# wtomin/MIMAMO-Net

Measured on AMD Instinct MI355X. Metric: face-frames/sec end-to-end (phase-diff + ResNet50 + 2-stream GRU), 64-frame clips, higher is better.
Workload: dtype f32

## Files before the change

### mimamo-net_amd/__init__.py

```python
__version__ = "0.1.0"

_LAZY = {
    "Phase_Difference_Extractor": ".phase_difference_extractor",
    "SCFpyr_PyTorch": ".scfpyr",
    "Steerable_Pyramid_Phase": ".phase_difference_extractor",
    "Resnet50_Extractor": ".resnet50_extractor",
    "Two_Stream_RNN": ".mimamo_net",
    "Tester": ".tester",
    "Snippet_Sampler": ".sampler",
    "Image_Sampler": ".sampler",
}


def __getattr__(name):
    if name in _LAZY:
        import importlib
        mod = importlib.import_module(_LAZY[name], __name__)
        return getattr(mod, name)
    raise AttributeError(name)
```

### mimamo-net_amd/csrc/conv.h

```cpp
#pragma once
#include "mm_common.h"

namespace mm {

struct ConvParams {
    const float* in;
    const float* w;
    const float* bias;
    const float* res;
    const float* post_scale;
    const float* post_shift;
    float* out;
    int B, H, W, Cin, in_cstride, in_coff;
    int Ho, Wo, Cout, out_cstride, out_coff;
    int res_cstride, res_coff;
    int res_rs, RH, RW;
    int kh, kw, stride, pad;
    int K, Kpad;
    int korder;
    int relu;
    int force_tile;
    int ablate;
    int Cin_real;
    int batch;
    int64_t in_bstride, w_bstride, out_bstride;
    int M, tiles_m, tiles_n;
    int m_end;
    int m_off;
    const float* in2;
    int H2, W2, C2, in2_cstride, in2_coff, stride2;
    int sched1x1;
    int no_sched;
    int use_panel;
    int x3;
    const unsigned short* w3;
    int64_t w3_plane;
    unsigned div_hw_mul, div_hw_sh, div_wo_mul, div_wo_sh;
    int hpool;
};

int conv_forward(const ConvParams& p, hipStream_t stream);
int bf16x3_split_weights(const float* w, unsigned short* out, int64_t n, hipStream_t stream);
bool conv_panel_supported(const ConvParams& p);
int conv_panel_forward(const ConvParams& p, hipStream_t stream);
int conv_panel_rows(const ConvParams& p);
int conv_panel_per_cu(const ConvParams& p);

int nchw_to_nhwc(const float* in, float* out, int64_t N, int C, int HW, int cstride, int coff, int cpad, hipStream_t s);
int nchw3_to_bordered_nhwc3(const float* in, float* out, int64_t N, int S, int pad, hipStream_t s);
int maxpool3x3s2(const float* in, float* out, int64_t N, int H, int W, int C, int Ho, int Wo, hipStream_t s);
int maxpool_reduce64(const float* in, const float* w, const float* bias, float* x_out, float* y_out, int64_t N, int H, int W, int Ho, int Wo,
                     int relu, hipStream_t s, int hp = 0);
int avgpool_hw(const float* in, float* out, int64_t N, int HW, int C, int out_cstride, int out_coff, int relu, hipStream_t s);
int wino_input_transform(const float* x, float* V, int B, int H, int W, int C, int m, hipStream_t s, int x_channels = 0);
int wino_output_transform(const float* M, const float* bias, float* y, int B, int H, int W, int Cout, int relu, int m, hipStream_t s);

int wino_gemm_output_fused(const float* V, const float* U, const float* bias, float* y, int B, int H, int W, int Cin, int Cout,
                           int relu, int shape, hipStream_t s, int generic_loop = 0);
int wino_gemm_output_fused_inc(const float* V, const float* U, const float* bias, const float* W2, const float* bias2, const float* res,
                               float* out, int B, int H, int W, int Cin, int Cout, int C2, int relu, hipStream_t s, int generic_loop = 0,
                               const float* next_w = nullptr, const float* next_bias = nullptr, float* next_out = nullptr, int shape = 0);
bool wino_fused_inc_supported(int64_t ntile, int Cin, int Cout, int C2);
int wino_gemm_output_fused_incproj(const float* V, const float* U, const float* bias, const float* W2, const float* bias2, const float* x,
                                   float* out, int B, int H, int W, int Cin, int Cout, int C2, int relu, hipStream_t s, int generic_loop = 0);
bool wino_fused_supported(int64_t ntile, int Cin, int Cout);

int gru_gates(const float* gi, int gi_stride, int gi_off, const float* gh, const float* bhh, const float* h_prev,
              int hp_stride, int hp_off, float* h_out, int out_stride, int out_off, int64_t Bt, int H, hipStream_t s);

}
```

### mimamo-net_amd/csrc/nets.hip

```cpp
#include <cmath>
#include <cstdlib>
#include <cstring>
#include <new>
#include "conv.h"

namespace mm {

struct Layer {
    float *w = nullptr, *bias = nullptr, *ps = nullptr, *pt = nullptr;
    float* wino_u = nullptr;
    float* wino_u4 = nullptr;
    int cin = 0, cin_p = 0, cout = 0, k = 1, stride = 1, pad = 0, K = 0, Kpad = 0, relu = 0, korder = 0;
    int wino_cin = 0;
    int tile = 0;
    unsigned short *w3 = nullptr, *wino_u4_3 = nullptr;
};

struct DeviceArena {
    std::vector<void*> ptrs;
    int upload(const std::vector<float>& h, float** out) {
        *out = nullptr;
        if (h.empty()) return MM_OK;
        void* d = nullptr;
        MM_HIP(hipMalloc(&d, h.size() * sizeof(float)));
        ptrs.push_back(d);
        MM_HIP(hipMemcpy(d, h.data(), h.size() * sizeof(float), hipMemcpyHostToDevice));
        *out = (float*)d;
        return MM_OK;
    }
    void release() {
        for (void* p : ptrs) (void)hipFree(p);
        ptrs.clear();
    }
};

struct BN {
    const float *gamma, *beta, *mean, *var;
};

static int make_layer(DeviceArena& A, Layer& L, const float* w, const float* bias, int cout, int cin, int k, int stride,
                      int pad, int relu, const BN* fold, const BN* post, float eps, bool wino = false, bool packed3 = false,
                      int wino_pad = 0) {
    if (packed3) {
        if (cin != 3) return MM_ERR_INVALID_ARG;
        const int RG = (k * 3 + 3) / 4 * 4;
        L.cin = 3; L.cin_p = 3; L.cout = cout; L.k = k; L.stride = stride; L.pad = 0; L.relu = relu;
        L.K = k * RG; L.Kpad = (L.K + 15) / 16 * 16; L.korder = 2;
        std::vector<float> hw((size_t)cout * L.Kpad, 0.f), hb(cout, 0.f);
        for (int o = 0; o < cout; ++o) {
            double sc = 1.0, sh = 0.0;
            if (fold) {
                sc = (double)fold->gamma[o] / std::sqrt((double)fold->var[o] + (double)eps);
                sh = (double)fold->beta[o] - (double)fold->mean[o] * sc;
            }
            for (int c = 0; c < 3; ++c)
                for (int r = 0; r < k; ++r)
                    for (int q = 0; q < k; ++q)
                        hw[(size_t)o * L.Kpad + r * RG + q * 3 + c] = (float)((double)w[(((size_t)o * 3 + c) * k + r) * k + q] * sc);
            hb[o] = (float)((bias ? (double)bias[o] : 0.0) * sc + sh);
        }
        int rc = A.upload(hw, &L.w);
        if (rc == MM_OK) rc = A.upload(hb, &L.bias);
        return rc;
    }
    L.cin = cin;
    L.cin_p = (cin + 3) / 4 * 4;
    L.cout = cout;
    L.k = k;
    L.stride = stride;
    L.pad = pad;
    L.relu = relu;
    L.K = k * k * L.cin_p;
    L.Kpad = (L.K + 15) / 16 * 16;
    L.korder = (k > 1 && L.cin_p % 16 == 0) ? 1 : 0;
    std::vector<float> hw((size_t)cout * L.Kpad, 0.f), hb(cout, 0.f);
    for (int o = 0; o < cout; ++o) {
        double sc = 1.0, sh = 0.0;
        if (fold) {
            sc = (double)fold->gamma[o] / std::sqrt((double)fold->var[o] + (double)eps);
            sh = (double)fold->beta[o] - (double)fold->mean[o] * sc;
        }
        for (int c = 0; c < cin; ++c)
            for (int r = 0; r < k; ++r)
                for (int s = 0; s < k; ++s)
                {
                    const size_t kidx = L.korder == 0 ? (size_t)(r * k + s) * L.cin_p + c
                                                      : ((size_t)((c / 16) * k + r) * k + s) * 16 + c % 16;
                    hw[(size_t)o * L.Kpad + kidx] = (float)((double)w[(((size_t)o * cin + c) * k + r) * k + s] * sc);
                }
        hb[o] = (float)((bias ? (double)bias[o] : 0.0) * sc + sh);
    }
    int rc = A.upload(hw, &L.w);
    if (rc == MM_OK) rc = A.upload(hb, &L.bias);
    const int wcin = wino_pad > 0 ? (cin + wino_pad - 1) / wino_pad * wino_pad : cin;
    if (rc == MM_OK && wino && k == 3 && stride == 1 && pad == 1 && wcin % 16 == 0 && cin >= 64 && cin % 4 == 0 && cout % 4 == 0) {
        L.wino_cin = wcin;
        static const double G[4][3] = {{1, 0, 0}, {0.5, 0.5, 0.5}, {0.5, -0.5, 0.5}, {0, 0, 1}};
        std::vector<float> hu((size_t)16 * cout * wcin, 0.f);
        for (int o = 0; o < cout; ++o) {
            const double sc = fold ? (double)fold->gamma[o] / std::sqrt((double)fold->var[o] + (double)eps) : 1.0;
            for (int c = 0; c < cin; ++c) {
                double g[3][3], t[4][3];
                for (int r = 0; r < 3; ++r)
                    for (int q = 0; q < 3; ++q) g[r][q] = (double)w[(((size_t)o * cin + c) * 3 + r) * 3 + q] * sc;
                for (int i = 0; i < 4; ++i)
                    for (int q = 0; q < 3; ++q) t[i][q] = G[i][0] * g[0][q] + G[i][1] * g[1][q] + G[i][2] * g[2][q];
                for (int i = 0; i < 4; ++i)
                    for (int j = 0; j < 4; ++j)
                        hu[((size_t)(i * 4 + j) * cout + o) * wcin + c] = (float)(t[i][0] * G[j][0] + t[i][1] * G[j][1] + t[i][2] * G[j][2]);
            }
        }
        rc = A.upload(hu, &L.wino_u);
        static const double G4[6][3] = {{0.25, 0, 0}, {-1.0 / 6, -1.0 / 6, -1.0 / 6}, {-1.0 / 6, 1.0 / 6, -1.0 / 6},
                                        {1.0 / 24, 1.0 / 12, 1.0 / 6}, {1.0 / 24, -1.0 / 12, 1.0 / 6}, {0, 0, 1}};
        std::vector<float> hu4((size_t)36 * cout * wcin, 0.f);
        for (int o = 0; o < cout && rc == MM_OK; ++o) {
            const double sc = fold ? (double)fold->gamma[o] / std::sqrt((double)fold->var[o] + (double)eps) : 1.0;
            for (int c = 0; c < cin; ++c) {
                double g[3][3], t[6][3];
                for (int r = 0; r < 3; ++r)
                    for (int q = 0; q < 3; ++q) g[r][q] = (double)w[(((size_t)o * cin + c) * 3 + r) * 3 + q] * sc;
                for (int i = 0; i < 6; ++i)
                    for (int q = 0; q < 3; ++q) t[i][q] = G4[i][0] * g[0][q] + G4[i][1] * g[1][q] + G4[i][2] * g[2][q];
                for (int i = 0; i < 6; ++i)
                    for (int j = 0; j < 6; ++j)
                        hu4[((size_t)(i * 6 + j) * cout + o) * wcin + c] = (float)(t[i][0] * G4[j][0] + t[i][1] * G4[j][1] + t[i][2] * G4[j][2]);
            }
        }
        if (rc == MM_OK) rc = A.upload(hu4, &L.wino_u4);
    }
    if (rc == MM_OK && post) {
        std::vector<float> ps(cout), pt(cout);
        for (int o = 0; o < cout; ++o) {
            const double sc = (double)post->gamma[o] / std::sqrt((double)post->var[o] + (double)eps);
            ps[o] = (float)sc;
            pt[o] = (float)((double)post->beta[o] - (double)post->mean[o] * sc);
        }
        rc = A.upload(ps, &L.ps);
        if (rc == MM_OK) rc = A.upload(pt, &L.pt);
    }
    return rc;
}

static int make_layer_dual(DeviceArena& A, Layer& L, const float* w1, const BN& bn1, int c1, const float* w2, const BN& bn2, int c2,
                           int cout, float eps) {
    if (c1 % 16 || c2 % 16) return MM_ERR_UNSUPPORTED;
    L.cin = c1; L.cin_p = c1; L.cout = cout; L.k = 1; L.stride = 1; L.pad = 0; L.relu = 1; L.korder = 0;
    L.K = L.Kpad = c1 + c2;
    std::vector<float> hw((size_t)cout * L.K), hb(cout);
    for (int o = 0; o < cout; ++o) {
        const double s1 = (double)bn1.gamma[o] / std::sqrt((double)bn1.var[o] + (double)eps);
        const double s2 = (double)bn2.gamma[o] / std::sqrt((double)bn2.var[o] + (double)eps);
        for (int c = 0; c < c1; ++c) hw[(size_t)o * L.K + c] = (float)((double)w1[(size_t)o * c1 + c] * s1);
        for (int c = 0; c < c2; ++c) hw[(size_t)o * L.K + c1 + c] = (float)((double)w2[(size_t)o * c2 + c] * s2);
        hb[o] = (float)(((double)bn1.beta[o] - (double)bn1.mean[o] * s1) + ((double)bn2.beta[o] - (double)bn2.mean[o] * s2));
    }
    int rc = A.upload(hw, &L.w);
    if (rc == MM_OK) rc = A.upload(hb, &L.bias);
    return rc;
}

constexpr int kX3MinK = 512;

static int run_layer(const Layer& L, const float* in, int B, int H, int W, int in_cstride, int in_coff, float* out,
                     int out_cstride, int out_coff, const float* res, int res_cstride, hipStream_t s, int* Ho_ = nullptr,
                     int* Wo_ = nullptr, int x3 = 0, int no_sched = 0, int hpool = 0, int use_panel = 0, int stride_ov = 0, int res_rs = 0,
                     int RH = 0, int RW = 0) {
    const int stride = stride_ov > 0 && L.k == 1 ? stride_ov : L.stride;
    ConvParams p;
    std::memset(&p, 0, sizeof(p));
    p.in = in; p.w = L.w; p.bias = L.bias; p.res = res; p.post_scale = L.ps; p.post_shift = L.pt; p.out = out;
    p.B = B; p.H = H; p.W = W; p.Cin = L.cin_p; p.in_cstride = in_cstride; p.in_coff = in_coff;
    p.Ho = (H + 2 * L.pad - L.k) / stride + 1;
    p.Wo = (W + 2 * L.pad - L.k) / stride + 1;
    p.Cout = L.cout; p.out_cstride = out_cstride; p.out_coff = out_coff;
    p.res_cstride = res_cstride; p.res_coff = 0;
    p.res_rs = res_rs; p.RH = RH; p.RW = RW;
    p.kh = L.k; p.kw = L.k; p.stride = stride; p.pad = L.pad;
    p.K = L.K; p.Kpad = L.Kpad; p.relu = L.relu; p.Cin_real = L.cin; p.korder = L.korder; p.force_tile = L.tile;
    p.x3 = x3 && L.k == 1 && L.Kpad >= kX3MinK;
    p.w3 = p.x3 ? L.w3 : nullptr; p.w3_plane = (int64_t)L.cout * L.Kpad;
    p.no_sched = no_sched;
    p.hpool = hpool;
    p.use_panel = use_panel;
    if (Ho_) *Ho_ = p.Ho;
    if (Wo_) *Wo_ = p.Wo;
    return conv_forward(p, s);
}

static int run_layer_dual(const Layer& L, const float* in, int B, int H, int W, const float* in2, int H2, int W2, int C2, int stride2,
                          float* out, hipStream_t s, int x3 = 0, int no_sched = 0) {
    ConvParams p;
    std::memset(&p, 0, sizeof(p));
    p.in = in; p.w = L.w; p.bias = L.bias; p.out = out;
    p.B = B; p.H = H; p.W = W; p.Cin = L.cin; p.in_cstride = L.cin; p.Ho = H; p.Wo = W;
    p.Cout = L.cout; p.out_cstride = L.cout; p.kh = 1; p.kw = 1; p.stride = 1;
    p.K = L.K; p.Kpad = L.Kpad; p.relu = 1; p.Cin_real = L.K;
    p.in2 = in2; p.H2 = H2; p.W2 = W2; p.C2 = C2; p.in2_cstride = C2; p.stride2 = stride2;
    p.x3 = x3 && L.Kpad >= kX3MinK;
    p.w3 = p.x3 ? L.w3 : nullptr; p.w3_plane = (int64_t)L.cout * L.Kpad;
    p.no_sched = no_sched;
    return conv_forward(p, s);
}

static int g_wino_fused_max_cin = 256;
static int g_wino_fused_shape = 0;

static int run_layer_wino(const Layer& L, const float* in, int B, int H, int W, float* out, float* V, float* M, int m, hipStream_t s,
                          const Layer* inc = nullptr, const float* inc_res = nullptr, float* inc_out = nullptr, bool inc_two_src = false,
                          int x3 = 0, int generic_loop = 0, int no_sched = 0, const Layer* next = nullptr, float* next_out = nullptr,
                          int inc_shape = 0) {
    const int mt = m == 5 ? 4 : m;
    const int TH = (H + mt - 1) / mt, TW = (W + mt - 1) / mt, npos = (mt + 2) * (mt + 2);
    const int64_t ntile = (int64_t)B * TH * TW;
    if (ntile > 0x7fffffff) return MM_ERR_INVALID_ARG;
    const bool fused = m == 5;
    if (fused) m = 4;
    const int wc = L.wino_cin;
    if (wc != L.cin_p && m != 4) return MM_ERR_UNSUPPORTED;
    if (!M && !(fused && wino_fused_supported(ntile, wc, L.cout))) return MM_ERR_UNSUPPORTED;
    if (inc && !(fused && inc->k == 1 && inc->stride == 1 && inc->Kpad == (inc_two_src ? 2 : 1) * L.cout && inc->korder == 0 && inc->relu &&
                 !inc->ps && (!inc_two_src || L.cout == 64) && wino_fused_inc_supported(ntile, wc, L.cout, inc->cout)))
        return MM_ERR_UNSUPPORTED;
    if (next && !(inc && !inc_two_src && L.cout == 64 && inc->cout == 256 && next_out && next->k == 1 && next->stride == 1 && next->pad == 0 &&
                  next->cin_p == 256 && next->Kpad == 256 && next->cout == 64 && next->korder == 0 && next->relu && !next->ps && next->bias))
        return MM_ERR_UNSUPPORTED;
    int rc = wino_input_transform(in, V, B, H, W, wc, m, s, L.cin_p);
    if (rc != MM_OK) return rc;
    if (inc && inc_two_src)
        return wino_gemm_output_fused_incproj(V, L.wino_u4, L.bias, inc->w, inc->bias, inc_res, inc_out, B, H, W, wc, L.cout, inc->cout,
                                              L.relu, s, generic_loop);
    if (inc)
        return wino_gemm_output_fused_inc(V, L.wino_u4, L.bias, inc->w, inc->bias, inc_res, inc_out, B, H, W, wc, L.cout, inc->cout,
                                          L.relu, s, generic_loop, next ? next->w : nullptr, next ? next->bias : nullptr, next_out, inc_shape);
    if (fused) {
        rc = wino_gemm_output_fused(V, L.wino_u4, L.bias, out, B, H, W, wc, L.cout, L.relu, g_wino_fused_shape, s, generic_loop);
        if (rc != MM_ERR_UNSUPPORTED) return rc;
    }
    if (!M) return MM_ERR_UNSUPPORTED;
    ConvParams p;
    std::memset(&p, 0, sizeof(p));
    p.in = V; p.w = m == 4 ? L.wino_u4 : L.wino_u; p.out = M;
    p.B = (int)ntile; p.H = 1; p.W = 1; p.Cin = wc; p.in_cstride = wc; p.Ho = 1; p.Wo = 1;
    p.Cout = L.cout; p.out_cstride = L.cout; p.kh = 1; p.kw = 1; p.stride = 1; p.K = wc; p.Kpad = wc; p.Cin_real = wc;
    p.batch = npos; p.in_bstride = ntile * wc; p.w_bstride = (int64_t)L.cout * wc; p.out_bstride = ntile * L.cout;
    p.x3 = x3 && wc >= kX3MinK;
    p.w3 = (p.x3 && m == 4) ? L.wino_u4_3 : nullptr; p.w3_plane = (int64_t)npos * L.cout * wc;
    p.no_sched = no_sched;
    rc = conv_forward(p, s);
    if (rc != MM_OK) return rc;
    return wino_output_transform(M, L.bias, out, B, H, W, L.cout, L.relu, m, s);
}

struct Bump {
    char* base;
    int64_t off = 0, cap;
    Bump(void* b, int64_t c) : base((char*)b), cap(c) {}
    float* take(int64_t floats) {
        const int64_t bytes = (floats * 4 + 255) / 256 * 256;
        float* p = (float*)(base + off);
        off += bytes;
        return p;
    }
    static int64_t size_of(int64_t floats) { return (floats * 4 + 255) / 256 * 256; }
};

static const int kStages[4][4] = {{3, 64, 256, 1}, {4, 128, 512, 2}, {6, 256, 1024, 2}, {3, 512, 2048, 2}};

struct Bottleneck {
    Layer proj, reduce, conv3, increase;
    Layer inc_proj;
    int proj_stride;
    bool has_proj;
};

}

struct mm_resnet50 {
    mm::DeviceArena arena;
    mm::Layer stem;
    mm::Layer stem3;
    std::vector<mm::Bottleneck> blocks;
    int ceil_mode;
    int winograd;
    int fuse_proj;
    int fuse_pool;
    int no_sched;
    int use_panel;
    int wf_generic;
    int precision;
    int fuse_next;
    int inc_shape;
    int fuse_inc;
    int stage_tail;
    int tail_fused;
    int device;
};

struct mm_head {
    mm::DeviceArena arena;
    std::vector<mm::Layer> mlp;
    int feat_dim, mlp_max;
    mm::Layer conv[6], fc1, fc2, transform, gru_ih[2], gru_hh[2][2], classifier;
    float* bhh[2][2];
    int winograd;
    int no_sched;
    int pc;
    int pcp;
    int device;
};

namespace mm {

static int64_t resnet_blob_floats() {
    int64_t n = 64 * 3 * 49 + 4 * 64;
    int cin = 64;
    for (auto& st : kStages)
        for (int b = 0; b < st[0]; ++b) {
            const int mid = st[1], cout = st[2];
            if (b == 0) n += (int64_t)cout * cin + 4 * cout;
            n += (int64_t)mid * cin + 4 * mid;
            n += (int64_t)mid * mid * 9 + 4 * mid;
            n += (int64_t)cout * mid + 4 * cout;
            cin = cout;
        }
    return n;
}

static const int64_t kRsIn4 = 224 * 224 * 4, kRsBig = 112 * 112 * 64, kRsMid = 56 * 56 * 128;
static const int64_t kRsWino = 36 * 14 * 14 * 64;

static const int kMlpPublished[3] = {2048, 256, 256};

static bool mlp_units_ok(int n_units, const int* units) {
    if (n_units < 2 || n_units > 16 || !units || units[n_units - 1] != 256) return false;
    for (int i = 0; i < n_units; ++i)
        if (units[i] <= 0 || units[i] % 4 || units[i] > 65536) return false;
    return true;
}

static bool phase_channels_ok(int pc) { return pc >= 2 && pc <= 256 && pc % 2 == 0; }
static int pad4(int c) { return (c + 3) / 4 * 4; }

static int64_t head_blob_floats(int n_units, const int* units, int pc = 24) {
    int64_t n = 0;
    auto lin = [&](int o, int i) { n += (int64_t)o * i + o; };
    auto bn = [&](int c) { n += 4 * c; };
    for (int i = 1; i < n_units; ++i) { lin(units[i], units[i - 1]); bn(units[i]); }
    const int ch[3][2] = {{pc, 64}, {64 + pc, 128}, {128, 256}};
    for (auto& c : ch) { n += (int64_t)c[1] * c[0] * 9 + c[1]; bn(c[1]); n += (int64_t)c[1] * c[1] * 9 + c[1]; bn(c[1]); }
    lin(256, 256); bn(256); lin(256, 256); bn(256); lin(1, 256); bn(1);
    lin(256, 512); bn(256);
    n += 4 * (384 * 256 + 384 * 128 + 384 + 384);
    lin(2, 256); bn(2);
    return n;
}

}

extern "C" {

int mm_conv2d_nhwc(const float* in, const float* w, const float* bias, const float* residual, const float* post_scale,
                   const float* post_shift, float* out, int B, int H, int W, int Cin, int in_cstride, int in_coff,
                   int Cout, int out_cstride, int out_coff, int res_cstride, int kh, int kw, int stride, int pad,
                   int relu, int tile, int korder, void* stream) {
    using namespace mm;
    if (!in || !w || !out || B < 0 || H <= 0 || W <= 0 || Cin <= 0 || Cout <= 0 || kh <= 0 || kw <= 0 || stride <= 0 ||
        pad < 0 || tile < 0)
        return MM_ERR_INVALID_ARG;
#ifdef MM_MEASURE
    if (tile > 2047) return MM_ERR_INVALID_ARG;
#else
    if (tile > 5) return MM_ERR_INVALID_ARG;
#endif
    if ((post_scale == nullptr) != (post_shift == nullptr)) return MM_ERR_INVALID_ARG;
    ConvParams p;
    std::memset(&p, 0, sizeof(p));
    p.in = in; p.w = w; p.bias = bias; p.res = residual; p.post_scale = post_scale; p.post_shift = post_shift; p.out = out;
    p.B = B; p.H = H; p.W = W; p.Cin = Cin; p.in_cstride = in_cstride; p.in_coff = in_coff;
    p.Ho = (H + 2 * pad - kh) / stride + 1;
    p.Wo = (W + 2 * pad - kw) / stride + 1;
    if (p.Ho <= 0 || p.Wo <= 0 || (int64_t)B * p.Ho * p.Wo > 0x7fffffff) return MM_ERR_INVALID_ARG;
    p.Cout = Cout; p.out_cstride = out_cstride; p.out_coff = out_coff; p.res_cstride = res_cstride;
    p.kh = kh; p.kw = kw; p.stride = stride; p.pad = pad;
    p.K = kh * kw * Cin; p.Kpad = (p.K + 15) / 16 * 16; p.relu = relu; p.force_tile = tile; p.korder = korder;
    {
        const char* cp = getenv("MM_CONV_PANEL");
        p.use_panel = cp ? (atoi(cp) == 1 ? 1 : atoi(cp) == 2 ? 2 : 0) : 0;
    }
    return conv_forward(p, (hipStream_t)stream);
}

int64_t mm_resnet50_blob_floats(void) { return mm::resnet_blob_floats(); }

int mm_resnet50_create(mm_resnet50_t** out, const float* blob, int64_t n_floats, int stride_on_first_1x1,
                       int maxpool_ceil_mode, float bn_eps) {
    using namespace mm;
    if (!out) return MM_ERR_INVALID_ARG;
    *out = nullptr;
    if (!blob || n_floats != resnet_blob_floats()) return MM_ERR_INVALID_ARG;
    int ndev = 0;
    if (hipGetDeviceCount(&ndev) != hipSuccess || ndev == 0) return MM_ERR_NO_DEVICE;
    mm_resnet50* h = new (std::nothrow) mm_resnet50();
    if (!h) return MM_ERR_INVALID_ARG;
    h->ceil_mode = maxpool_ceil_mode;
    h->device = current_device_or(0);
    const float* p = blob;
    int rc = MM_OK;
    h->winograd = 1;
    h->precision = 0;
    {
        const char* wk = getenv("MM_WF_KSL");
        h->wf_generic = wk ? atoi(wk) == 0 : 0;
        const char* cs = getenv("MM_CONV_SCHED");
        h->no_sched = cs ? atoi(cs) == 0 : 0;
        const char* cp = getenv("MM_CONV_PANEL");
        h->use_panel = cp ? (atoi(cp) == 1 ? 1 : atoi(cp) == 2 ? 2 : 0) : 0;
        const char* fp = getenv("MM_FUSE_PROJ");
        h->fuse_proj = fp ? atoi(fp) : 1;
        const char* fpl = getenv("MM_FUSE_POOL");
        h->fuse_pool = fpl ? atoi(fpl) : 2;
        const char* fi = getenv("MM_FUSE_INC");
        h->fuse_inc = fi ? atoi(fi) : 3;
        const char* fn = getenv("MM_FUSE_NEXT");
        h->fuse_next = fn ? atoi(fn) : 0;
        const char* is = getenv("MM_INC1_SHAPE");
        h->inc_shape = is ? atoi(is) : 0;
        const char* tl = getenv("MM_STAGE_TAIL");
        h->stage_tail = tl ? atoi(tl) != 0 : 1;
        const char* tf = getenv("MM_STAGE_TAIL_FUSED");
        h->tail_fused = tf ? atoi(tf) & 3 : 3;
    }
    auto conv_bn = [&](Layer& L, int cout, int cin, int k, int stride, int pad, int relu) {
        const float* w = p;
        p += (int64_t)cout * cin * k * k;
        BN bn{p, p + cout, p + 2 * cout, p + 3 * cout};
        p += 4 * cout;
        if (rc == MM_OK) rc = make_layer(h->arena, L, w, nullptr, cout, cin, k, stride, pad, relu, &bn, nullptr, bn_eps, true);
    };
    {
        const float* w = p;
        BN bn{p + 64 * 3 * 49, p + 64 * 3 * 49 + 64, p + 64 * 3 * 49 + 128, p + 64 * 3 * 49 + 192};
        rc = make_layer(h->arena, h->stem3, w, nullptr, 64, 3, 7, 2, 0, 1, &bn, nullptr, bn_eps, false, true);
    }
    conv_bn(h->stem, 64, 3, 7, 2, 3, 1);
#ifdef MM_MEASURE
    if (const char* st = getenv("MM_STEM_TILE")) {
        const int t = atoi(st);
        if (t >= 0 && t <= 4) h->stem.tile = h->stem3.tile = t;
    }
#endif
    int cin = 64;
    for (auto& st : kStages)
        for (int b = 0; b < st[0]; ++b) {
            const int mid = st[1], cout = st[2], s = b == 0 ? st[3] : 1;
            const int s1 = stride_on_first_1x1 ? s : 1, s3 = stride_on_first_1x1 ? 1 : s;
            h->blocks.emplace_back();
            Bottleneck& B = h->blocks.back();
            B.has_proj = b == 0;
            B.proj_stride = s;
            const float* w_proj = p;
            if (b == 0) conv_bn(B.proj, cout, cin, 1, s, 0, 0);
            conv_bn(B.reduce, mid, cin, 1, s1, 0, 1);
            conv_bn(B.conv3, mid, mid, 3, s3, 1, 1);
            const float* w_inc = p;
            conv_bn(B.increase, cout, mid, 1, 1, 0, 1);
            if (b == 0 && rc == MM_OK) {
                const float* q1 = w_inc + (int64_t)cout * mid;
                const float* q2 = w_proj + (int64_t)cout * cin;
                const BN bn1{q1, q1 + cout, q1 + 2 * cout, q1 + 3 * cout}, bn2{q2, q2 + cout, q2 + 2 * cout, q2 + 3 * cout};
                const int rd = make_layer_dual(h->arena, B.inc_proj, w_inc, bn1, mid, w_proj, bn2, cin, cout, bn_eps);
                if (rd != MM_OK && rd != MM_ERR_UNSUPPORTED) rc = rd;
            }
            cin = cout;
        }
    if (rc != MM_OK) {
        h->arena.release();
        delete h;
        return rc;
    }
    *out = h;
    return MM_OK;
}

int mm_resnet50_destroy(mm_resnet50_t* h) {
    if (!h) return MM_OK;
    h->arena.release();
    delete h;
    return MM_OK;
}

int64_t mm_resnet50_workspace_bytes(mm_resnet50_t* h, int64_t batch) {
    using namespace mm;
    if (!h || batch < 0) return MM_ERR_INVALID_ARG;
    return Bump::size_of(batch * kRsIn4) + 3 * Bump::size_of(batch * kRsBig) + 2 * Bump::size_of(batch * kRsMid) +
           2 * Bump::size_of(batch * kRsWino);
}

int mm_resnet50_set_winograd(mm_resnet50_t* h, int enable) {
    if (!h) return MM_ERR_INVALID_ARG;
    if (enable != 0 && enable != 1 && enable != 2 && enable != 4 && enable != 5) return MM_ERR_INVALID_ARG;
    h->winograd = enable;
#ifdef MM_MEASURE
    const char* mc = getenv("MM_WF_MAX_CIN");
    if (mc) mm::g_wino_fused_max_cin = atoi(mc);
    const char* sh = getenv("MM_WINO_FUSED_SHAPE");
    mm::g_wino_fused_shape = sh ? atoi(sh) : 0;
#endif
    return MM_OK;
}

static int ensure_x3_weights(mm_resnet50_t* h) {
    using namespace mm;
    const char* e = getenv("MM_X3_PRESPLIT");
    if (!e || atoi(e) != 1) return MM_OK;
    auto split = [&](const float* w, int64_t n, unsigned short** out) -> int {
        if (*out || !w || n <= 0 || n % 16) return MM_OK;
        void* d = nullptr;
        MM_HIP(hipMalloc(&d, (size_t)n * 3 * sizeof(unsigned short)));
        h->arena.ptrs.push_back(d);
        const int rc = bf16x3_split_weights(w, (unsigned short*)d, n, nullptr);
        if (rc != MM_OK) return rc;
        *out = (unsigned short*)d;
        return MM_OK;
    };
    for (auto& Bk : h->blocks) {
        for (Layer* L : {&Bk.proj, &Bk.reduce, &Bk.increase, &Bk.inc_proj})
            if (L->w && L->k == 1 && L->Kpad >= kX3MinK && L->cout % 256 == 0) {
                const int rc = split(L->w, (int64_t)L->cout * L->Kpad, &L->w3);
                if (rc != MM_OK) return rc;
            }
        Layer& C = Bk.conv3;
        if (C.wino_u4 && C.wino_cin >= kX3MinK && C.cout % 256 == 0) {
            const int rc = split(C.wino_u4, (int64_t)36 * C.cout * C.wino_cin, &C.wino_u4_3);
            if (rc != MM_OK) return rc;
        }
    }
    MM_HIP(hipDeviceSynchronize());
    return MM_OK;
}

int mm_resnet50_set_precision(mm_resnet50_t* h, int mode) {
    if (!h || (mode != 0 && mode != 1)) return MM_ERR_INVALID_ARG;
    if (mode == 1) {
        MM_CHECK_DEVICE(h);
        const int rc = ensure_x3_weights(h);
        if (rc != MM_OK) return rc;
    }
    h->precision = mode;
    return MM_OK;
}

int mm_resnet50_forward(mm_resnet50_t* h, const float* images, int nchw, int64_t batch, float* out, void* workspace,
                        int64_t workspace_bytes, void* stream_) {
    using namespace mm;
    if (!h || batch < 0 || (batch > 0 && (!images || !out || !workspace))) return MM_ERR_INVALID_ARG;
    if (batch == 0) return MM_OK;
    if (batch > 40000) return MM_ERR_INVALID_ARG;
    MM_CHECK_DEVICE(h);
    if (workspace_bytes < mm_resnet50_workspace_bytes(h, batch)) return MM_ERR_WORKSPACE;
    hipStream_t s = (hipStream_t)stream_;
    const int B = (int)batch;
    Bump ws(workspace, workspace_bytes);
    float* in4 = ws.take(batch * kRsIn4);
    float* big[3] = {ws.take(batch * kRsBig), ws.take(batch * kRsBig), ws.take(batch * kRsBig)};
    float* y1 = ws.take(batch * kRsMid);
    float* y2 = ws.take(batch * kRsMid);
    float* wv = ws.take(batch * kRsWino);
    float* wm = ws.take(batch * kRsWino);
    int rc;
    const float* x0 = images;
    int H = 224, W = 224, Ho, Wo;
    const mm::Layer& R0 = h->blocks.front().reduce;
    const bool pooled_reduce = h->fuse_pool && R0.k == 1 && R0.stride == 1 && R0.pad == 0 && R0.cin_p == 64 && R0.cout == 64 && R0.Kpad == 64 &&
                               R0.korder == 0 && !R0.ps;
    const bool hpool = pooled_reduce && h->fuse_pool >= 2 && nchw;
    if (nchw) {
        if (nchw == 1) {
            rc = nchw3_to_bordered_nhwc3(images, in4, batch, 224, 3, s);
            if (rc != MM_OK) return rc;
            x0 = in4;
        }
        rc = run_layer(h->stem3, x0, B, 230, 230, 3, 0, big[0], 64, 0, nullptr, 0, s, &Ho, &Wo, 0, h->no_sched, hpool);
    } else {
        rc = run_layer(h->stem, x0, B, H, W, 4, 0, big[0], 64, 0, nullptr, 0, s, &Ho, &Wo, 0, h->no_sched);
    }
    if (rc != MM_OK) return rc;
    if (Ho != 112 || Wo != 112) return MM_ERR_UNSUPPORTED;
    H = Ho; W = Wo;
    if (h->ceil_mode) {
        Ho = (H - 3 + 1) / 2 + 1; Wo = (W - 3 + 1) / 2 + 1;
        if ((Ho - 1) * 2 >= H) --Ho;
        if ((Wo - 1) * 2 >= W) --Wo;
    } else {
        Ho = (H - 3) / 2 + 1; Wo = (W - 3) / 2 + 1;
    }
    if (pooled_reduce)
        rc = maxpool_reduce64(big[0], R0.w, R0.bias, big[1], y1, batch, H, W, Ho, Wo, R0.relu, s, hpool);
    else
        rc = maxpool3x3s2(big[0], big[1], batch, H, W, 64, Ho, Wo, s);
    if (rc != MM_OK) return rc;
    H = Ho; W = Wo;
    int xi = 1;
    int C = 64;
    const int x3 = h->precision == 1, ns = h->no_sched;
    bool reduce_done = false;
    bool xc = false;
    for (size_t bi = 0; bi < h->blocks.size(); ++bi) {
        const Bottleneck& Bk = h->blocks[bi];
        const Bottleneck* Nx = bi + 1 < h->blocks.size() ? &h->blocks[bi + 1] : nullptr;
        float* x = big[xi];
        float* sc = big[(xi + 1) % 3];
        float* o = big[(xi + 2) % 3];
        int H1, W1, H2, W2, H3, W3;
        const float* resid = x;
        const bool dual = Bk.has_proj && h->fuse_proj && Bk.inc_proj.w;
        const bool tail_blk = !Bk.has_proj && Nx && Nx->has_proj && Nx->proj_stride == 2 && Nx->reduce.k == 1 && Nx->reduce.stride == 2 &&
                              Nx->reduce.pad == 0 && Nx->proj.k == 1 && Nx->proj.pad == 0 && Bk.increase.k == 1 && Bk.increase.stride == 1 &&
                              Bk.increase.pad == 0;
        bool tail = tail_blk && h->stage_tail && !h->use_panel;
        const bool tail_unfuse = tail_blk && !(h->tail_fused & (Bk.conv3.cout == 64 ? 1 : 2));
        const int sov = xc ? 1 : 0;
        if (Bk.has_proj && !dual) {
            rc = run_layer(Bk.proj, x, B, H, W, C, 0, sc, Bk.proj.cout, 0, nullptr, 0, s, nullptr, nullptr, x3, ns, 0, 0, sov);
            if (rc != MM_OK) return rc;
            resid = sc;
        }
        if ((pooled_reduce && bi == 0) || reduce_done) {
            H1 = H; W1 = W;
            reduce_done = false;
        } else {
            rc = run_layer(Bk.reduce, x, B, H, W, C, 0, y1, Bk.reduce.cout, 0, nullptr, 0, s, &H1, &W1, x3, ns, 0, 0, sov);
            if (rc != MM_OK) return rc;
        }
        const int wm_ = h->winograd == 1 ? (Bk.conv3.cin <= g_wino_fused_max_cin ? 5 : 4) : h->winograd;
        const int wt_ = wm_ == 5 ? 4 : wm_;
        bool inc_done = false;
        if (wm_ && Bk.conv3.wino_u &&
            (int64_t)(wt_ + 2) * (wt_ + 2) * ((H1 + wt_ - 1) / wt_) * ((W1 + wt_ - 1) / wt_) * Bk.conv3.cin <= kRsWino) {
            rc = MM_ERR_UNSUPPORTED;
            if (wm_ == 5 && h->fuse_inc && !Bk.has_proj && !tail_unfuse && (Bk.conv3.cout == 64 || h->fuse_inc >= 3)) {
                const bool nx = h->fuse_next && Bk.conv3.cout == 64 && Nx && !Nx->has_proj && Nx->reduce.stride == 1;
                if (nx) {
                    rc = run_layer_wino(Bk.conv3, y1, B, H1, W1, nullptr, wv, nullptr, 5, s, &Bk.increase, x, o, false, 0, h->wf_generic, 0, &Nx->reduce, y1,
                                        h->inc_shape);
                    reduce_done = rc == MM_OK;
                }
                if (!nx || rc == MM_ERR_UNSUPPORTED)
                    rc = run_layer_wino(Bk.conv3, y1, B, H1, W1, nullptr, wv, nullptr, 5, s, &Bk.increase, x, o, false, 0, h->wf_generic, 0, nullptr, nullptr,
                                        h->inc_shape);
                inc_done = rc == MM_OK;
            } else if (wm_ == 5 && h->fuse_inc >= 2 && dual && Bk.proj_stride == 1 && C == Bk.conv3.cout && H1 == H && W1 == W) {
                rc = run_layer_wino(Bk.conv3, y1, B, H1, W1, nullptr, wv, nullptr, 5, s, &Bk.inc_proj, x, o, true, 0, h->wf_generic);
                inc_done = rc == MM_OK;
            }
            if (rc == MM_ERR_UNSUPPORTED) rc = run_layer_wino(Bk.conv3, y1, B, H1, W1, y2, wv, wm, wm_, s, nullptr, nullptr, nullptr, false, x3, h->wf_generic, ns);
            H2 = H1; W2 = W1;
        } else {
            rc = run_layer(Bk.conv3, y1, B, H1, W1, Bk.reduce.cout, 0, y2, Bk.conv3.cout, 0, nullptr, 0, s, &H2, &W2, 0, ns);
        }
        if (rc != MM_OK) return rc;
        if (inc_done) {
            H3 = H2; W3 = W2;
            tail = false;
        } else if (dual) {
            rc = run_layer_dual(Bk.inc_proj, y2, B, H2, W2, x, H, W, C, xc ? 1 : Bk.proj_stride, o, s, x3, ns);
            H3 = H2; W3 = W2;
        } else if (tail) {
            rc = run_layer(Bk.increase, y2, B, H2, W2, Bk.conv3.cout, 0, o, Bk.increase.cout, 0, resid, Bk.increase.cout, s, &H3, &W3, x3, ns, 0,
                           h->use_panel, 2, 2, H2, W2);
        } else {
            rc = run_layer(Bk.increase, y2, B, H2, W2, Bk.conv3.cout, 0, o, Bk.increase.cout, 0, resid, Bk.increase.cout, s, &H3, &W3, x3, ns, 0, h->use_panel);
        }
        if (rc != MM_OK) return rc;
        H = H3; W = W3; C = Bk.increase.cout;
        xc = tail;
        xi = (xi + 2) % 3;
    }
    if (H != 7 || W != 7) return MM_ERR_UNSUPPORTED;
    return avgpool_hw(big[xi], out, batch, H * W, C, C, 0, 1, s);
}

int64_t mm_head_blob_floats(void) { return mm::head_blob_floats(3, mm::kMlpPublished); }

int64_t mm_head_blob_floats_mlp(int n_units, const int* units) {
    return mm::mlp_units_ok(n_units, units) ? mm::head_blob_floats(n_units, units) : (int64_t)MM_ERR_INVALID_ARG;
}

int mm_head_create(mm_head_t** out, const float* blob, int64_t n_floats) {
    return mm_head_create_mlp(out, blob, n_floats, 3, mm::kMlpPublished);
}

int mm_head_create_mlp(mm_head_t** out, const float* blob, int64_t n_floats, int n_units, const int* units) {
    return mm_head_create_cfg(out, blob, n_floats, n_units, units, 12);
}

int64_t mm_head_blob_floats_cfg(int n_units, const int* units, int num_phase) {
    if (!mm::mlp_units_ok(n_units, units) || num_phase < 1) return (int64_t)MM_ERR_INVALID_ARG;
    if (!mm::phase_channels_ok(2 * num_phase)) return (int64_t)MM_ERR_UNSUPPORTED;
    return mm::head_blob_floats(n_units, units, 2 * num_phase);
}

int mm_head_create_cfg(mm_head_t** out, const float* blob, int64_t n_floats, int n_units, const int* units, int num_phase) {
    using namespace mm;
    if (!out) return MM_ERR_INVALID_ARG;
    *out = nullptr;
    const int pc = 2 * num_phase;
    if (!mlp_units_ok(n_units, units)) return MM_ERR_INVALID_ARG;
    if (num_phase < 1) return MM_ERR_INVALID_ARG;
    if (!phase_channels_ok(pc)) return MM_ERR_UNSUPPORTED;
    if (!blob || n_floats != head_blob_floats(n_units, units, pc)) return MM_ERR_INVALID_ARG;
    int ndev = 0;
    if (hipGetDeviceCount(&ndev) != hipSuccess || ndev == 0) return MM_ERR_NO_DEVICE;
    mm_head* h = new (std::nothrow) mm_head();
    if (!h) return MM_ERR_INVALID_ARG;
    h->device = current_device_or(0);
    h->pc = pc;
    h->pcp = pad4(pc);
    const float eps = 1e-5f;
    const float* p = blob;
    int rc = MM_OK;
    auto take = [&](int64_t n) { const float* q = p; p += n; return q; };
    auto take_bn = [&](int c) { BN b{p, p + c, p + 2 * c, p + 3 * c}; p += 4 * c; return b; };
    auto lin_bn_relu = [&](Layer& L, int o, int i) {
        const float* w = take((int64_t)o * i); const float* b = take(o); BN bn = take_bn(o);
        if (rc == MM_OK) rc = make_layer(h->arena, L, w, b, o, i, 1, 1, 0, 1, &bn, nullptr, eps);
    };
    auto conv_bn_relu = [&](Layer& L, int o, int i, int stride, bool wino) {
        const float* w = take((int64_t)o * i * 9); const float* b = take(o); BN bn = take_bn(o);
        if (rc == MM_OK) rc = make_layer(h->arena, L, w, b, o, i, 3, stride, 1, 1, &bn, nullptr, eps, wino && i <= 128, false, 64);
    };
    auto lin_relu_bn = [&](Layer& L, int o, int i) {
        const float* w = take((int64_t)o * i); const float* b = take(o); BN bn = take_bn(o);
        if (rc == MM_OK) rc = make_layer(h->arena, L, w, b, o, i, 1, 1, 0, 1, nullptr, &bn, eps);
    };
    {
        const char* e = getenv("MM_HEAD_WINOGRAD");
        h->winograd = e ? atoi(e) : 1;
        const char* cs = getenv("MM_CONV_SCHED");
        h->no_sched = cs ? atoi(cs) == 0 : 0;
    }
    h->feat_dim = units[0];
    h->mlp_max = 256;
    h->mlp.resize(n_units - 1);
    for (int i = 1; i < n_units; ++i) {
        lin_bn_relu(h->mlp[i - 1], units[i], units[i - 1]);
        if (units[i] > h->mlp_max) h->mlp_max = units[i];
    }
    const int ch[3][2] = {{pc, 64}, {64 + pc, 128}, {128, 256}};
    for (int i = 0; i < 3; ++i) {
        conv_bn_relu(h->conv[2 * i], ch[i][1], ch[i][0], 1, i >= 1);
        conv_bn_relu(h->conv[2 * i + 1], ch[i][1], ch[i][1], 2, false);
    }
    lin_relu_bn(h->fc1, 256, 256);
    lin_relu_bn(h->fc2, 256, 256);
    take(256 + 1); take_bn(1);
    lin_relu_bn(h->transform, 256, 512);
    for (int l = 0; l < 2 && rc == MM_OK; ++l) {
        std::vector<float> wih(768 * 256), bih(768);
        for (int d = 0; d < 2; ++d) {
            const float* w_ih = take(384 * 256); const float* w_hh = take(384 * 128);
            const float* b_ih = take(384); const float* b_hh = take(384);
            std::memcpy(wih.data() + (size_t)d * 384 * 256, w_ih, sizeof(float) * 384 * 256);
            std::memcpy(bih.data() + (size_t)d * 384, b_ih, sizeof(float) * 384);
            if (rc == MM_OK) rc = make_layer(h->arena, h->gru_hh[l][d], w_hh, b_hh, 384, 128, 1, 1, 0, 0, nullptr, nullptr, eps);
            std::vector<float> bh(b_hh, b_hh + 384);
            if (rc == MM_OK) rc = h->arena.upload(bh, &h->bhh[l][d]);
        }
        if (rc == MM_OK) rc = make_layer(h->arena, h->gru_ih[l], wih.data(), bih.data(), 768, 256, 1, 1, 0, 0, nullptr, nullptr, eps);
    }
    {
        const float* w = take(2 * 256); const float* b = take(2); BN bn = take_bn(2);
        if (rc == MM_OK) rc = make_layer(h->arena, h->classifier, w, b, 2, 256, 1, 1, 0, 0, &bn, nullptr, eps);
    }
    if (rc == MM_OK && p - blob != n_floats) rc = MM_ERR_INVALID_ARG;
    if (rc != MM_OK) {
        h->arena.release();
        delete h;
        return rc;
    }
    *out = h;
    return MM_OK;
}

int mm_head_destroy(mm_head_t* h) {
    if (!h) return MM_OK;
    h->arena.release();
    delete h;
    return MM_OK;
}

namespace {
struct HeadWs {
    int64_t p0n, a0, cat, a1, a2, a3, a4, pool, fc1, m1, feat, f, gi, gh, l0, l1, wv;
};
HeadWs head_sizes(int64_t N, int64_t T, int64_t mlp_max, bool wino, int pc) {
    HeadWs s;
    s.p0n = N * 48 * 48 * pc; s.a0 = N * 48 * 48 * 64; s.cat = N * 24 * 24 * (64 + pc); s.a1 = N * 24 * 24 * 128;
    s.a2 = N * 12 * 12 * 128; s.a3 = N * 12 * 12 * 256; s.a4 = N * 6 * 6 * 256; s.pool = N * 256; s.fc1 = N * 256;
    s.m1 = 2 * N * mlp_max; s.feat = N * 512; s.f = N * 256; s.gi = N * 768; s.gh = T * 384; s.l0 = N * 256; s.l1 = N * 256;
    s.wv = wino ? N * 36 * 36 * 128 : 0;
    return s;
}
}

int64_t mm_head_workspace_bytes(mm_head_t* h, int64_t bs, int64_t T) {
    using mm::Bump;
    if (!h || bs < 0 || T < 0) return MM_ERR_INVALID_ARG;
    const HeadWs s = head_sizes(bs * T, T, h->mlp_max, h->winograd != 0, h->pcp);
    const int64_t all[] = {s.p0n, s.a0, s.cat, s.a1, s.a2, s.a3, s.a4, s.pool, s.fc1, s.m1, s.feat, s.f, s.gi, s.gh, s.l0, s.l1, s.wv};
    int64_t tot = 0;
    for (int64_t v : all) tot += Bump::size_of(v);
    return tot;
}

int mm_head_forward(mm_head_t* h, const float* phase_0, const float* phase_1, int phase_nhwc, const float* rgb,
                    int64_t bs, int64_t T, float* out, void* workspace, int64_t workspace_bytes, void* stream_) {
    using namespace mm;
    if (!h || bs < 0 || T < 0) return MM_ERR_INVALID_ARG;
    const int64_t N64 = bs * T;
    if (N64 == 0) return MM_OK;
    if (!phase_0 || !phase_1 || !rgb || !out || !workspace || N64 > 400000) return MM_ERR_INVALID_ARG;
    if (workspace_bytes < mm_head_workspace_bytes(h, bs, T)) return MM_ERR_WORKSPACE;
    MM_CHECK_DEVICE(h);
    hipStream_t s = (hipStream_t)stream_;
    const int N = (int)N64;
    const HeadWs z = head_sizes(N64, T, h->mlp_max, h->winograd != 0, h->pcp);
    Bump ws(workspace, workspace_bytes);
    float* p0n = ws.take(z.p0n); float* a0 = ws.take(z.a0); float* cat = ws.take(z.cat); float* a1 = ws.take(z.a1);
    float* a2 = ws.take(z.a2); float* a3 = ws.take(z.a3); float* a4 = ws.take(z.a4); float* pool = ws.take(z.pool);
    float* fc1 = ws.take(z.fc1); float* m1 = ws.take(z.m1); float* feat = ws.take(z.feat); float* f = ws.take(z.f);
    float* gi = ws.take(z.gi); float* gh = ws.take(z.gh); float* l0 = ws.take(z.l0); float* l1 = ws.take(z.l1);
    float* wv = ws.take(z.wv);
    int rc;
#define MM_TRY(x) do { rc = (x); if (rc != MM_OK) return rc; } while (0)
    const float* x0 = phase_0;
    const int pc = h->pc, pcp = h->pcp, catc = 64 + pcp;
    if (phase_nhwc && pcp != pc) return MM_ERR_UNSUPPORTED;
    if (!phase_nhwc) {
        MM_TRY(nchw_to_nhwc(phase_0, p0n, N64, pc, 48 * 48, pcp, 0, pcp, s));
        MM_TRY(nchw_to_nhwc(phase_1, cat, N64, pc, 24 * 24, catc, 64, pcp, s));
        x0 = p0n;
    } else if (phase_nhwc == 2) {
        cat = const_cast<float*>(phase_1);
    } else {
        MM_HIP(hipMemcpy2DAsync(cat + 64, catc * sizeof(float), phase_1, pc * sizeof(float), pc * sizeof(float),
                                (size_t)N64 * 24 * 24, hipMemcpyDeviceToDevice, s));
    }
    MM_TRY(run_layer(h->conv[0], x0, N, 48, 48, pcp, 0, a0, 64, 0, nullptr, 0, s, nullptr, nullptr, 0, h->no_sched));
    MM_TRY(run_layer(h->conv[1], a0, N, 48, 48, 64, 0, cat, catc, 0, nullptr, 0, s, nullptr, nullptr, 0, h->no_sched));
    rc = MM_ERR_UNSUPPORTED;
    if (h->winograd && h->conv[2].wino_u4) rc = run_layer_wino(h->conv[2], cat, N, 24, 24, a1, wv, nullptr, 5, s);
    if (rc == MM_ERR_UNSUPPORTED) rc = run_layer(h->conv[2], cat, N, 24, 24, catc, 0, a1, 128, 0, nullptr, 0, s, nullptr, nullptr, 0, h->no_sched);
    if (rc != MM_OK) return rc;
    MM_TRY(run_layer(h->conv[3], a1, N, 24, 24, 128, 0, a2, 128, 0, nullptr, 0, s, nullptr, nullptr, 0, h->no_sched));
    rc = MM_ERR_UNSUPPORTED;
    if (h->winograd && h->conv[4].wino_u4) rc = run_layer_wino(h->conv[4], a2, N, 12, 12, a3, wv, nullptr, 5, s);
    if (rc == MM_ERR_UNSUPPORTED) rc = run_layer(h->conv[4], a2, N, 12, 12, 128, 0, a3, 256, 0, nullptr, 0, s, nullptr, nullptr, 0, h->no_sched);
    if (rc != MM_OK) return rc;
    MM_TRY(run_layer(h->conv[5], a3, N, 12, 12, 256, 0, a4, 256, 0, nullptr, 0, s, nullptr, nullptr, 0, h->no_sched));
    MM_TRY(avgpool_hw(a4, pool, N64, 36, 256, 256, 0, 0, s));
    MM_TRY(run_layer(h->fc1, pool, N, 1, 1, 256, 0, fc1, 256, 0, nullptr, 0, s, nullptr, nullptr, 0, h->no_sched));
    MM_TRY(run_layer(h->fc2, fc1, N, 1, 1, 256, 0, feat, 512, 256, nullptr, 0, s, nullptr, nullptr, 0, h->no_sched));
    {
        const float* xin = rgb;
        int cin = h->feat_dim;
        for (size_t i = 0; i < h->mlp.size(); ++i) {
            const bool last = i + 1 == h->mlp.size();
            float* dst = last ? feat : m1 + (i & 1) * N64 * h->mlp_max;
            MM_TRY(run_layer(h->mlp[i], xin, N, 1, 1, cin, 0, dst, last ? 512 : h->mlp[i].cout, 0, nullptr, 0, s, nullptr, nullptr, 0, h->no_sched));
            xin = dst;
            cin = h->mlp[i].cout;
        }
    }
    MM_TRY(run_layer(h->transform, feat, N, 1, 1, 512, 0, f, 256, 0, nullptr, 0, s, nullptr, nullptr, 0, h->no_sched));
    const int Ti = (int)T, S = (int)bs;
    const float* x = f;
    float* lay[2] = {l0, l1};
    for (int l = 0; l < 2; ++l) {
        MM_TRY(run_layer(h->gru_ih[l], x, N, 1, 1, 256, 0, gi, 768, 0, nullptr, 0, s, nullptr, nullptr, 0, h->no_sched));
        for (int d = 0; d < 2; ++d) {
            for (int step = 0; step < S; ++step) {
                const int t = d == 0 ? step : S - 1 - step;
                float* hout = lay[l] + (int64_t)t * Ti * 256;
                const float* git = gi + (int64_t)t * Ti * 768;
                if (step == 0) {
                    MM_TRY(gru_gates(git, 768, d * 384, nullptr, h->bhh[l][d], nullptr, 0, 0, hout, 256, d * 128, Ti, 128, s));
                } else {
                    const int tp = d == 0 ? t - 1 : t + 1;
                    const float* hprev = lay[l] + (int64_t)tp * Ti * 256;
                    MM_TRY(run_layer(h->gru_hh[l][d], hprev, Ti, 1, 1, 256, d * 128, gh, 384, 0, nullptr, 0, s, nullptr, nullptr, 0, h->no_sched));
                    MM_TRY(gru_gates(git, 768, d * 384, gh, nullptr, hprev, 256, d * 128, hout, 256, d * 128, Ti, 128, s));
                }
            }
        }
        x = lay[l];
    }
    MM_TRY(run_layer(h->classifier, l1, N, 1, 1, 256, 0, out, 2, 0, nullptr, 0, s, nullptr, nullptr, 0, h->no_sched));
#undef MM_TRY
    return MM_OK;
}

}
```

### mimamo-net_amd/csrc/wino_fused.hip

```cpp
#include <cstdio>
#include <cstdlib>
#include <type_traits>
#include "conv.h"

namespace mm {

typedef float f32x4v __attribute__((ext_vector_type(4)));
#ifndef MM_WF_NT_STORES
#define MM_WF_NT_STORES 1
#endif
__device__ __forceinline__ void inc_store(const f32x4v& v, float* dst) {
    if (MM_WF_NT_STORES) __builtin_nontemporal_store(v, reinterpret_cast<f32x4v*>(dst));
    else *reinterpret_cast<f32x4v*>(dst) = v;
}

struct WinoFusedParams {
    const float* V;
    const float* U;
    const float* bias;
    float* out;
    int ntile, K, Cout, B, H, W, TH, TW, relu, tiles_n;
    float at_cols[24];
    const float* w2;
    const float* bias2;
    const float* res;
    int C2;
    const float* w3;
    const float* bias3;
    float* out3;
    int generic_loop;
    int ablate;
};

#ifndef MM_INC3_PAIR
#define MM_INC3_PAIR 0
#endif
__host__ __device__ constexpr int inc3_lds_bytes(int ring_bytes) {
    return MM_INC3_PAIR && ring_bytes < (128 * 128 + 4 * 8 * 512 + 512) * 4 ? (128 * 128 + 4 * 8 * 512 + 512) * 4 : ring_bytes;
}

__device__ constexpr float kAt[4][6] = {{1, 1, 1, 1, 1, 0}, {0, 1, -1, 2, -2, 0}, {0, 1, 1, 4, 4, 0}, {0, 1, -1, 8, -8, 1}};
static constexpr float kAtHost[4][6] = {{1, 1, 1, 1, 1, 0}, {0, 1, -1, 2, -2, 0}, {0, 1, 1, 4, 4, 0}, {0, 1, -1, 8, -8, 1}};

template <int NBUF, int WGM, int INC = 0, int WGN = 2, int KSL = 0, int NEXT = 0>
__global__ void __launch_bounds__(WGM * WGN * 64) __attribute__((amdgpu_waves_per_eu(2, 2)))
wino_fused_kernel(const WinoFusedParams p) {
    constexpr int NW = WGN * WGM, BM = 16 * WGM, BN = 32 * WGN, KS = 64;
    constexpr int ROWS = BM + BN;
    constexpr int NIA = BM / (4 * NW), NIB = BN / (4 * NW);
    constexpr int NL = NIA + NIB;
    constexpr int SLAB_BYTES = ROWS * KS * 4;
    extern __shared__ __attribute__((aligned(16))) float lds[];

    const int tid = threadIdx.x, lane = tid & 63, wave = __builtin_amdgcn_readfirstlane(tid >> 6);
    const int wm = wave / WGN, wn = wave % WGN;
    const int l16 = lane & 15, lg = lane >> 4;
    const int logical = xcd_contiguous(blockIdx.x, gridDim.x);
    const int tile_m = logical / p.tiles_n, tile_n = logical - tile_m * p.tiles_n;
    const int m_base = tile_m * BM, n_base = tile_n * BN;
#ifdef MM_MEASURE
    const int m_load = (p.ablate & 1) ? (m_base & 1023) : m_base;
#else
    const int m_load = m_base;
#endif
    static_assert(BM % (4 * NW) == 0 && BN % (4 * NW) == 0, "whole 1 KB pieces per wave");
    const int K = p.K, kslabs = K / KS;

    unsigned va[NIA], vb[NIB];
#pragma unroll
    for (int it = 0; it < NIA; ++it) {
        const int row = (it * NW + wave) * 4 + (lane >> 4);
        va[it] = (unsigned)((m_load + row) * K + (((lane & 15) ^ (row & 15)) << 2)) * 4u;
    }
#pragma unroll
    for (int it = 0; it < NIB; ++it) {
        const int row = (it * NW + wave) * 4 + (lane >> 4);
        vb[it] = (unsigned)((n_base + row) * K + (((lane & 15) ^ (row & 15)) << 2)) * 4u;
    }
    const unsigned lds0 = (unsigned)(uintptr_t)(__attribute__((address_space(3))) float*)lds;
    const unsigned plane_a = (unsigned)p.ntile * (unsigned)K * 4u;
    const unsigned plane_b = (unsigned)p.Cout * (unsigned)K * 4u;
    auto dma1 = [&](const __amdgpu_buffer_rsrc_t& rsrc, unsigned voff, unsigned lds_byte) {
        const unsigned m0v = __builtin_amdgcn_readfirstlane(lds_byte);
        unsigned keep;
        asm volatile("s_mov_b32 %0, m0\n\ts_mov_b32 m0, %3\n\ts_nop 0\n\tbuffer_load_dwordx4 %1, %2, 0 offen lds\n\ts_mov_b32 m0, %0"
                     : "=&s"(keep) : "v"(voff), "s"(rsrc), "s"(m0v) : "memory");
    };
    const char* pv = reinterpret_cast<const char*>(p.V);
    const char* pu = reinterpret_cast<const char*>(p.U);
    const int64_t step_a = 6 * (int64_t)plane_a, step_b = 6 * (int64_t)plane_b;
    const int64_t back_a = 35 * (int64_t)plane_a, back_b = 35 * (int64_t)plane_b;
    unsigned rec_a = plane_a, rec_b = plane_b;
    unsigned koff = 0;
    int d_q = 0, d_r = 0, d_ks = 0, d_buf = 0;
    auto dma_next = [&]() {
        const __amdgpu_buffer_rsrc_t ra = __builtin_amdgcn_make_buffer_rsrc(const_cast<char*>(pv), 0, rec_a, 0x00020000);
        const __amdgpu_buffer_rsrc_t rb = __builtin_amdgcn_make_buffer_rsrc(const_cast<char*>(pu), 0, rec_b, 0x00020000);
        const unsigned base = __builtin_amdgcn_readfirstlane(lds0 + (unsigned)d_buf * SLAB_BYTES + (unsigned)wave * 1024u);
        unsigned keep;
        if constexpr (NIA == 2 && NIB == 4) {
            asm volatile("s_mov_b32 %0, m0\n\t"
                         "s_add_u32 m0, %9, %10\n\ts_nop 0\n\tbuffer_load_dwordx4 %1, %7, 0 offen lds\n\t"
                         "s_add_u32 m0, %9, %11\n\ts_nop 0\n\tbuffer_load_dwordx4 %2, %7, 0 offen lds\n\t"
                         "s_add_u32 m0, %9, %12\n\ts_nop 0\n\tbuffer_load_dwordx4 %3, %8, 0 offen lds\n\t"
                         "s_add_u32 m0, %9, %13\n\ts_nop 0\n\tbuffer_load_dwordx4 %4, %8, 0 offen lds\n\t"
                         "s_add_u32 m0, %9, %14\n\ts_nop 0\n\tbuffer_load_dwordx4 %5, %8, 0 offen lds\n\t"
                         "s_add_u32 m0, %9, %15\n\ts_nop 0\n\tbuffer_load_dwordx4 %6, %8, 0 offen lds\n\t"
                         "s_mov_b32 m0, %0"
                         : "=&s"(keep)
                         : "v"(va[0] + koff), "v"(va[1] + koff), "v"(vb[0] + koff), "v"(vb[1] + koff), "v"(vb[2] + koff), "v"(vb[3] + koff),
                           "s"(ra), "s"(rb), "s"(base), "n"(0), "n"(NW * 1024), "n"(BM * KS * 4), "n"(BM * KS * 4 + NW * 1024),
                           "n"(BM * KS * 4 + 2 * NW * 1024), "n"(BM * KS * 4 + 3 * NW * 1024)
                         : "memory", "scc");
        } else if constexpr (NIA == 1 && NIB == 4) {
            asm volatile("s_mov_b32 %0, m0\n\t"
                         "s_add_u32 m0, %8, %9\n\ts_nop 0\n\tbuffer_load_dwordx4 %1, %6, 0 offen lds\n\t"
                         "s_add_u32 m0, %8, %10\n\ts_nop 0\n\tbuffer_load_dwordx4 %2, %7, 0 offen lds\n\t"
                         "s_add_u32 m0, %8, %11\n\ts_nop 0\n\tbuffer_load_dwordx4 %3, %7, 0 offen lds\n\t"
                         "s_add_u32 m0, %8, %12\n\ts_nop 0\n\tbuffer_load_dwordx4 %4, %7, 0 offen lds\n\t"
                         "s_add_u32 m0, %8, %13\n\ts_nop 0\n\tbuffer_load_dwordx4 %5, %7, 0 offen lds\n\t"
                         "s_mov_b32 m0, %0"
                         : "=&s"(keep)
                         : "v"(va[0] + koff), "v"(vb[0] + koff), "v"(vb[1] + koff), "v"(vb[2] + koff), "v"(vb[3] + koff),
                           "s"(ra), "s"(rb), "s"(base), "n"(0), "n"(BM * KS * 4), "n"(BM * KS * 4 + NW * 1024),
                           "n"(BM * KS * 4 + 2 * NW * 1024), "n"(BM * KS * 4 + 3 * NW * 1024)
                         : "memory", "scc");
        } else {
            static_assert(NIA == 2 && NIB == 2, "piece counts of the workgroup shapes");
            asm volatile("s_mov_b32 %0, m0\n\t"
                         "s_add_u32 m0, %7, %8\n\ts_nop 0\n\tbuffer_load_dwordx4 %1, %5, 0 offen lds\n\t"
                         "s_add_u32 m0, %7, %9\n\ts_nop 0\n\tbuffer_load_dwordx4 %2, %5, 0 offen lds\n\t"
                         "s_add_u32 m0, %7, %10\n\ts_nop 0\n\tbuffer_load_dwordx4 %3, %6, 0 offen lds\n\t"
                         "s_add_u32 m0, %7, %11\n\ts_nop 0\n\tbuffer_load_dwordx4 %4, %6, 0 offen lds\n\t"
                         "s_mov_b32 m0, %0"
                         : "=&s"(keep)
                         : "v"(va[0] + koff), "v"(va[1] + koff), "v"(vb[0] + koff), "v"(vb[1] + koff), "s"(ra), "s"(rb), "s"(base), "n"(0),
                           "n"(NW * 1024), "n"(BM * KS * 4), "n"(BM * KS * 4 + NW * 1024)
                         : "memory", "scc");
        }
        koff += KS * 4u;
        if (++d_ks == kslabs) {
            d_ks = 0;
            koff = 0;
            pv += step_a;
            pu += step_b;
            if (++d_r == 6) {
                d_r = 0;
                pv -= back_a;
                pu -= back_b;
                if (++d_q == 6) rec_a = rec_b = 0;
            }
        }
        d_buf = d_buf == NBUF - 1 ? 0 : d_buf + 1;
    };

    int fa[4], fb0[4], fb1[4];
#pragma unroll
    for (int j = 0; j < 4; ++j) {
        const int sw = ((lg + 4 * j) ^ l16) << 2;
        fa[j] = (wm * 16 + l16) * KS + sw;
        fb0[j] = (BM + wn * 32 + l16) * KS + sw;
        fb1[j] = (BM + wn * 32 + 16 + l16) * KS + sw;
    }

    f32x4v Y[4][4][2], T[4][2], M[2][2];
#pragma unroll
    for (int a = 0; a < 4; ++a)
#pragma unroll
        for (int c = 0; c < 2; ++c) {
            T[a][c] = f32x4v{0.f, 0.f, 0.f, 0.f};
#pragma unroll
            for (int b = 0; b < 4; ++b) Y[a][b][c] = f32x4v{0.f, 0.f, 0.f, 0.f};
        }
    M[0][0] = M[0][1] = M[1][0] = M[1][1] = f32x4v{0.f, 0.f, 0.f, 0.f};

    auto update_t = [&](const f32x4v (&Mx)[2], auto rtag) {
        constexpr int r = decltype(rtag)::value;
#pragma unroll
        for (int pp = 0; pp < 4; ++pp) {
            const float c = kAt[pp][r];
            if (c == 0.f) continue;
#pragma unroll
            for (int cb = 0; cb < 2; ++cb)
#pragma unroll
                for (int e = 0; e < 4; ++e) T[pp][cb][e] = c == 1.f ? T[pp][cb][e] + Mx[cb][e] : fmaf(c, Mx[cb][e], T[pp][cb][e]);
        }
    };
    auto update_y = [&](int qc) {
#pragma unroll
        for (int qq = 0; qq < 4; ++qq) {
            const float c = p.at_cols[qc * 4 + qq];
#pragma unroll
            for (int pp = 0; pp < 4; ++pp)
#pragma unroll
                for (int cb = 0; cb < 2; ++cb)
#pragma unroll
                    for (int e = 0; e < 4; ++e) Y[pp][qq][cb][e] = fmaf(c, T[pp][cb][e], Y[pp][qq][cb][e]);
        }
#pragma unroll
        for (int pp = 0; pp < 4; ++pp)
#pragma unroll
            for (int cb = 0; cb < 2; ++cb) T[pp][cb] = f32x4v{0.f, 0.f, 0.f, 0.f};
    };

    int buf = 0;
    auto slab = [&](f32x4v (&Mc)[2], auto first_tag) {
        constexpr bool first = decltype(first_tag)::value;
        asm volatile("s_waitcnt vmcnt(%0) lgkmcnt(0)\n\ts_barrier" :: "n"((NBUF - 2) * NL) : "memory");
        dma_next();
        const float* sl = lds + buf * (ROWS * KS);
        float4 a[4], b0[4], b1[4];
#pragma unroll
        for (int j = 0; j < 4; ++j) {
            a[j] = *reinterpret_cast<const float4*>(sl + fa[j]);
            b0[j] = *reinterpret_cast<const float4*>(sl + fb0[j]);
            b1[j] = *reinterpret_cast<const float4*>(sl + fb1[j]);
        }
        if (first) Mc[0] = Mc[1] = f32x4v{0.f, 0.f, 0.f, 0.f};
        if constexpr (INC) {
#pragma unroll
            for (int j = 0; j < 4; ++j) {
                Mc[0] = __builtin_amdgcn_mfma_f32_16x16x4f32(b0[j].x, a[j].x, Mc[0], 0, 0, 0);
                Mc[1] = __builtin_amdgcn_mfma_f32_16x16x4f32(b1[j].x, a[j].x, Mc[1], 0, 0, 0);
                Mc[0] = __builtin_amdgcn_mfma_f32_16x16x4f32(b0[j].y, a[j].y, Mc[0], 0, 0, 0);
                Mc[1] = __builtin_amdgcn_mfma_f32_16x16x4f32(b1[j].y, a[j].y, Mc[1], 0, 0, 0);
                Mc[0] = __builtin_amdgcn_mfma_f32_16x16x4f32(b0[j].z, a[j].z, Mc[0], 0, 0, 0);
                Mc[1] = __builtin_amdgcn_mfma_f32_16x16x4f32(b1[j].z, a[j].z, Mc[1], 0, 0, 0);
                Mc[0] = __builtin_amdgcn_mfma_f32_16x16x4f32(b0[j].w, a[j].w, Mc[0], 0, 0, 0);
                Mc[1] = __builtin_amdgcn_mfma_f32_16x16x4f32(b1[j].w, a[j].w, Mc[1], 0, 0, 0);
            }
        } else {
#pragma unroll
        for (int j = 0; j < 4; ++j) {
            Mc[0] = __builtin_amdgcn_mfma_f32_16x16x4f32(a[j].x, b0[j].x, Mc[0], 0, 0, 0);
            Mc[1] = __builtin_amdgcn_mfma_f32_16x16x4f32(a[j].x, b1[j].x, Mc[1], 0, 0, 0);
            Mc[0] = __builtin_amdgcn_mfma_f32_16x16x4f32(a[j].y, b0[j].y, Mc[0], 0, 0, 0);
            Mc[1] = __builtin_amdgcn_mfma_f32_16x16x4f32(a[j].y, b1[j].y, Mc[1], 0, 0, 0);
            Mc[0] = __builtin_amdgcn_mfma_f32_16x16x4f32(a[j].z, b0[j].z, Mc[0], 0, 0, 0);
            Mc[1] = __builtin_amdgcn_mfma_f32_16x16x4f32(a[j].z, b1[j].z, Mc[1], 0, 0, 0);
            Mc[0] = __builtin_amdgcn_mfma_f32_16x16x4f32(a[j].w, b0[j].w, Mc[0], 0, 0, 0);
            Mc[1] = __builtin_amdgcn_mfma_f32_16x16x4f32(a[j].w, b1[j].w, Mc[1], 0, 0, 0);
        }
        }
        buf = buf == NBUF - 1 ? 0 : buf + 1;
    };

    if constexpr (KSL > 0) {
        static_assert(NBUF == 3 && (6 * KSL) % NBUF == 0, "a column's slabs cover the ring a whole number of times");
        constexpr int NSL = 6 * KSL;
        typedef __attribute__((address_space(3))) const f32x4v* lds_f4;
        constexpr bool FAR2 = (NBUF - 1) * SLAB_BYTES > 65535;
        unsigned ab[4], bb0[4], bb1[4], ab2[4], bb0_2[4], bb1_2[4];
#pragma unroll
        for (int j = 0; j < 4; ++j) {
            ab[j] = lds0 + (unsigned)fa[j] * 4u;
            bb0[j] = lds0 + (unsigned)fb0[j] * 4u;
            bb1[j] = lds0 + (unsigned)fb1[j] * 4u;
            if constexpr (FAR2) {
                ab2[j] = ab[j] + (NBUF - 1) * SLAB_BYTES;
                bb0_2[j] = bb0[j] + (NBUF - 1) * SLAB_BYTES;
                bb1_2[j] = bb1[j] + (NBUF - 1) * SLAB_BYTES;
                asm volatile("" : "+v"(ab2[j]), "+v"(bb0_2[j]), "+v"(bb1_2[j]));
            }
        }
        auto frag = [&](const unsigned (&lo)[4], const unsigned (&hi)[4], int j, auto buf_tag) -> f32x4v {
            constexpr int BUF = decltype(buf_tag)::value;
            if constexpr (FAR2 && BUF == NBUF - 1) return *(lds_f4)(uintptr_t)(hi[j]);
            else return *(lds_f4)(uintptr_t)(lo[j] + BUF * SLAB_BYTES);
        };
        const unsigned dbase = __builtin_amdgcn_readfirstlane(lds0 + (unsigned)wave * 1024u);
        int dq = 0;
        auto dma_c = [&](auto d_tag) {
            constexpr int D = decltype(d_tag)::value % NSL;
            constexpr int DBUF = D % NBUF, DKS = D % KSL, DR = D / KSL;
            constexpr unsigned SB = DBUF * SLAB_BYTES;
            const __amdgpu_buffer_rsrc_t ra = __builtin_amdgcn_make_buffer_rsrc(const_cast<char*>(pv), 0, rec_a, 0x00020000);
            const __amdgpu_buffer_rsrc_t rb = __builtin_amdgcn_make_buffer_rsrc(const_cast<char*>(pu), 0, rec_b, 0x00020000);
            const unsigned ko = __builtin_amdgcn_readfirstlane(DKS * KS * 4);
            unsigned keep;
#ifdef MM_MEASURE
            if (p.ablate & 128) {
                rec_a = rec_b = 0;
            }
#endif
            if constexpr (NIA == 2 && NIB == 4) {
                asm volatile("s_mov_b32 %0, m0\n\t"
                             "s_add_u32 m0, %9, %10\n\ts_nop 0\n\tbuffer_load_dwordx4 %1, %7, %16 offen lds\n\t"
                             "s_add_u32 m0, %9, %11\n\ts_nop 0\n\tbuffer_load_dwordx4 %2, %7, %16 offen lds\n\t"
                             "s_add_u32 m0, %9, %12\n\ts_nop 0\n\tbuffer_load_dwordx4 %3, %8, %16 offen lds\n\t"
                             "s_add_u32 m0, %9, %13\n\ts_nop 0\n\tbuffer_load_dwordx4 %4, %8, %16 offen lds\n\t"
                             "s_add_u32 m0, %9, %14\n\ts_nop 0\n\tbuffer_load_dwordx4 %5, %8, %16 offen lds\n\t"
                             "s_add_u32 m0, %9, %15\n\ts_nop 0\n\tbuffer_load_dwordx4 %6, %8, %16 offen lds\n\t"
                             "s_mov_b32 m0, %0"
                             : "=&s"(keep)
                             : "v"(va[0]), "v"(va[1]), "v"(vb[0]), "v"(vb[1]), "v"(vb[2]), "v"(vb[3]),
                               "s"(ra), "s"(rb), "s"(dbase), "n"(SB), "n"(SB + NW * 1024), "n"(SB + BM * KS * 4), "n"(SB + BM * KS * 4 + NW * 1024),
                               "n"(SB + BM * KS * 4 + 2 * NW * 1024), "n"(SB + BM * KS * 4 + 3 * NW * 1024), "s"(ko)
                             : "memory", "scc");
            } else if constexpr (NIA == 1 && NIB == 4) {
                asm volatile("s_mov_b32 %0, m0\n\t"
                             "s_add_u32 m0, %8, %9\n\ts_nop 0\n\tbuffer_load_dwordx4 %1, %6, %14 offen lds\n\t"
                             "s_add_u32 m0, %8, %10\n\ts_nop 0\n\tbuffer_load_dwordx4 %2, %7, %14 offen lds\n\t"
                             "s_add_u32 m0, %8, %11\n\ts_nop 0\n\tbuffer_load_dwordx4 %3, %7, %14 offen lds\n\t"
                             "s_add_u32 m0, %8, %12\n\ts_nop 0\n\tbuffer_load_dwordx4 %4, %7, %14 offen lds\n\t"
                             "s_add_u32 m0, %8, %13\n\ts_nop 0\n\tbuffer_load_dwordx4 %5, %7, %14 offen lds\n\t"
                             "s_mov_b32 m0, %0"
                             : "=&s"(keep)
                             : "v"(va[0]), "v"(vb[0]), "v"(vb[1]), "v"(vb[2]), "v"(vb[3]),
                               "s"(ra), "s"(rb), "s"(dbase), "n"(SB), "n"(SB + BM * KS * 4), "n"(SB + BM * KS * 4 + NW * 1024),
                               "n"(SB + BM * KS * 4 + 2 * NW * 1024), "n"(SB + BM * KS * 4 + 3 * NW * 1024), "s"(ko)
                             : "memory", "scc");
            } else {
                static_assert(NIA == 2 && NIB == 2, "piece counts of the workgroup shapes");
                asm volatile("s_mov_b32 %0, m0\n\t"
                             "s_add_u32 m0, %7, %8\n\ts_nop 0\n\tbuffer_load_dwordx4 %1, %5, %12 offen lds\n\t"
                             "s_add_u32 m0, %7, %9\n\ts_nop 0\n\tbuffer_load_dwordx4 %2, %5, %12 offen lds\n\t"
                             "s_add_u32 m0, %7, %10\n\ts_nop 0\n\tbuffer_load_dwordx4 %3, %6, %12 offen lds\n\t"
                             "s_add_u32 m0, %7, %11\n\ts_nop 0\n\tbuffer_load_dwordx4 %4, %6, %12 offen lds\n\t"
                             "s_mov_b32 m0, %0"
                             : "=&s"(keep)
                             : "v"(va[0]), "v"(va[1]), "v"(vb[0]), "v"(vb[1]), "s"(ra), "s"(rb), "s"(dbase), "n"(SB),
                               "n"(SB + NW * 1024), "n"(SB + BM * KS * 4), "n"(SB + BM * KS * 4 + NW * 1024), "s"(ko)
                             : "memory", "scc");
            }
            if constexpr (DKS == KSL - 1) {
                pv += step_a;
                pu += step_b;
                if constexpr (DR == 5) {
                    pv -= back_a;
                    pu -= back_b;
                    if (++dq == 6) rec_a = rec_b = 0;
                }
            }
        };
#ifndef MM_WF_HOOK
#define MM_WF_HOOK 1
#endif
        auto slab_c = [&](auto n_tag, auto&& hook) {
            constexpr int N = decltype(n_tag)::value;
            constexpr int BUF = N % NBUF;
            constexpr bool first = N % KSL == 0;
            f32x4v (&Mc)[2] = M[(N / KSL) & 1];
            asm volatile("s_waitcnt vmcnt(%0) lgkmcnt(0)\n\ts_barrier" :: "n"((NBUF - 2) * NL) : "memory");
            dma_c(std::integral_constant<int, N + NBUF - 1>());
            if (first) Mc[0] = Mc[1] = f32x4v{0.f, 0.f, 0.f, 0.f};
            if constexpr (INC) {
#pragma unroll
                for (int hh = 0; hh < 2; ++hh) {
                    f32x4v a[2], b0[2], b1[2];
#pragma unroll
                    for (int j = 0; j < 2; ++j) {
                        a[j] = frag(ab, ab2, 2 * hh + j, std::integral_constant<int, BUF>());
                        b0[j] = frag(bb0, bb0_2, 2 * hh + j, std::integral_constant<int, BUF>());
                        b1[j] = frag(bb1, bb1_2, 2 * hh + j, std::integral_constant<int, BUF>());
                    }
#pragma unroll
                    for (int j = 0; j < 2; ++j) {
                        Mc[0] = __builtin_amdgcn_mfma_f32_16x16x4f32(b0[j].x, a[j].x, Mc[0], 0, 0, 0);
                        Mc[1] = __builtin_amdgcn_mfma_f32_16x16x4f32(b1[j].x, a[j].x, Mc[1], 0, 0, 0);
                        Mc[0] = __builtin_amdgcn_mfma_f32_16x16x4f32(b0[j].y, a[j].y, Mc[0], 0, 0, 0);
                        Mc[1] = __builtin_amdgcn_mfma_f32_16x16x4f32(b1[j].y, a[j].y, Mc[1], 0, 0, 0);
                        Mc[0] = __builtin_amdgcn_mfma_f32_16x16x4f32(b0[j].z, a[j].z, Mc[0], 0, 0, 0);
                        Mc[1] = __builtin_amdgcn_mfma_f32_16x16x4f32(b1[j].z, a[j].z, Mc[1], 0, 0, 0);
                        Mc[0] = __builtin_amdgcn_mfma_f32_16x16x4f32(b0[j].w, a[j].w, Mc[0], 0, 0, 0);
                        Mc[1] = __builtin_amdgcn_mfma_f32_16x16x4f32(b1[j].w, a[j].w, Mc[1], 0, 0, 0);
                    }
                    __builtin_amdgcn_sched_barrier(0);
                }
            } else {
            f32x4v a[4], b0[4], b1[4];
#pragma unroll
            for (int j = 0; j < 4; ++j) {
                a[j] = frag(ab, ab2, j, std::integral_constant<int, BUF>());
                b0[j] = frag(bb0, bb0_2, j, std::integral_constant<int, BUF>());
                b1[j] = frag(bb1, bb1_2, j, std::integral_constant<int, BUF>());
            }
            if (MM_WF_HOOK) {
                __builtin_amdgcn_sched_barrier(0);
                hook();
                __builtin_amdgcn_sched_barrier(0);
            }
            if constexpr (false) {
#pragma unroll
                for (int j = 0; j < 4; ++j) {
                    Mc[0] = __builtin_amdgcn_mfma_f32_16x16x4f32(b0[j].x, a[j].x, Mc[0], 0, 0, 0);
                    Mc[1] = __builtin_amdgcn_mfma_f32_16x16x4f32(b1[j].x, a[j].x, Mc[1], 0, 0, 0);
                    Mc[0] = __builtin_amdgcn_mfma_f32_16x16x4f32(b0[j].y, a[j].y, Mc[0], 0, 0, 0);
                    Mc[1] = __builtin_amdgcn_mfma_f32_16x16x4f32(b1[j].y, a[j].y, Mc[1], 0, 0, 0);
                    Mc[0] = __builtin_amdgcn_mfma_f32_16x16x4f32(b0[j].z, a[j].z, Mc[0], 0, 0, 0);
                    Mc[1] = __builtin_amdgcn_mfma_f32_16x16x4f32(b1[j].z, a[j].z, Mc[1], 0, 0, 0);
                    Mc[0] = __builtin_amdgcn_mfma_f32_16x16x4f32(b0[j].w, a[j].w, Mc[0], 0, 0, 0);
                    Mc[1] = __builtin_amdgcn_mfma_f32_16x16x4f32(b1[j].w, a[j].w, Mc[1], 0, 0, 0);
                }
            } else {
#pragma unroll
                for (int j = 0; j < 4; ++j) {
                    Mc[0] = __builtin_amdgcn_mfma_f32_16x16x4f32(a[j].x, b0[j].x, Mc[0], 0, 0, 0);
                    Mc[1] = __builtin_amdgcn_mfma_f32_16x16x4f32(a[j].x, b1[j].x, Mc[1], 0, 0, 0);
                    Mc[0] = __builtin_amdgcn_mfma_f32_16x16x4f32(a[j].y, b0[j].y, Mc[0], 0, 0, 0);
                    Mc[1] = __builtin_amdgcn_mfma_f32_16x16x4f32(a[j].y, b1[j].y, Mc[1], 0, 0, 0);
                    Mc[0] = __builtin_amdgcn_mfma_f32_16x16x4f32(a[j].z, b0[j].z, Mc[0], 0, 0, 0);
                    Mc[1] = __builtin_amdgcn_mfma_f32_16x16x4f32(a[j].z, b1[j].z, Mc[1], 0, 0, 0);
                    Mc[0] = __builtin_amdgcn_mfma_f32_16x16x4f32(a[j].w, b0[j].w, Mc[0], 0, 0, 0);
                    Mc[1] = __builtin_amdgcn_mfma_f32_16x16x4f32(a[j].w, b1[j].w, Mc[1], 0, 0, 0);
                }
            }
            }
        };
        auto nothing = []() {};
        auto position = [&](auto r_tag, auto&& hook) {
            constexpr int r = decltype(r_tag)::value;
            slab_c(std::integral_constant<int, r * KSL>(), hook);
            if constexpr (KSL > 1) slab_c(std::integral_constant<int, r * KSL + 1>(), nothing);
            if constexpr (KSL > 2) {
                slab_c(std::integral_constant<int, r * KSL + 2>(), nothing);
                slab_c(std::integral_constant<int, r * KSL + 3>(), nothing);
            }
            static_assert(KSL == 1 || KSL == 2 || KSL == 4, "K = 64, 128 or 256");
        };
        dma_c(std::integral_constant<int, 0>());
        dma_c(std::integral_constant<int, 1>());
        for (int q = 0; q < 6; ++q) {
            if constexpr (MM_WF_HOOK && INC == 0) {
            position(std::integral_constant<int, 0>(), [&]() { update_t(M[1], std::integral_constant<int, 5>()); update_y(q == 0 ? 0 : q - 1); });
            position(std::integral_constant<int, 1>(), [&]() { update_t(M[0], std::integral_constant<int, 0>()); });
            position(std::integral_constant<int, 2>(), [&]() { update_t(M[1], std::integral_constant<int, 1>()); });
            position(std::integral_constant<int, 3>(), [&]() { update_t(M[0], std::integral_constant<int, 2>()); });
            position(std::integral_constant<int, 4>(), [&]() { update_t(M[1], std::integral_constant<int, 3>()); });
            position(std::integral_constant<int, 5>(), [&]() { update_t(M[0], std::integral_constant<int, 4>()); });
            } else {
#ifdef MM_MEASURE
            if (p.ablate & 4) {
                position(std::integral_constant<int, 0>(), nothing);
                position(std::integral_constant<int, 1>(), nothing);
                position(std::integral_constant<int, 2>(), nothing);
                position(std::integral_constant<int, 3>(), nothing);
                position(std::integral_constant<int, 4>(), nothing);
                position(std::integral_constant<int, 5>(), nothing);
                Y[0][0][0] += M[0][0] + M[1][0]; Y[0][0][1] += M[0][1] + M[1][1];
                continue;
            }
#endif
            position(std::integral_constant<int, 0>(), nothing);
            update_t(M[1], std::integral_constant<int, 5>());
            update_y(q == 0 ? 0 : q - 1);
            position(std::integral_constant<int, 1>(), nothing);
            update_t(M[0], std::integral_constant<int, 0>());
            position(std::integral_constant<int, 2>(), nothing);
            update_t(M[1], std::integral_constant<int, 1>());
            position(std::integral_constant<int, 3>(), nothing);
            update_t(M[0], std::integral_constant<int, 2>());
            position(std::integral_constant<int, 4>(), nothing);
            update_t(M[1], std::integral_constant<int, 3>());
            position(std::integral_constant<int, 5>(), nothing);
            update_t(M[0], std::integral_constant<int, 4>());
            }
        }
    } else {
#pragma unroll
    for (int i = 0; i < NBUF - 1; ++i) dma_next();
    for (int q = 0; q < 6; ++q) {
        slab(M[0], std::true_type());
        for (int ks = 1; ks < kslabs; ++ks) slab(M[0], std::false_type());
        update_t(M[1], std::integral_constant<int, 5>());
        update_y(q == 0 ? 0 : q - 1);
        slab(M[1], std::true_type());
        for (int ks = 1; ks < kslabs; ++ks) slab(M[1], std::false_type());
        update_t(M[0], std::integral_constant<int, 0>());
        slab(M[0], std::true_type());
        for (int ks = 1; ks < kslabs; ++ks) slab(M[0], std::false_type());
        update_t(M[1], std::integral_constant<int, 1>());
        slab(M[1], std::true_type());
        for (int ks = 1; ks < kslabs; ++ks) slab(M[1], std::false_type());
        update_t(M[0], std::integral_constant<int, 2>());
        slab(M[0], std::true_type());
        for (int ks = 1; ks < kslabs; ++ks) slab(M[0], std::false_type());
        update_t(M[1], std::integral_constant<int, 3>());
        slab(M[1], std::true_type());
        for (int ks = 1; ks < kslabs; ++ks) slab(M[1], std::false_type());
        update_t(M[0], std::integral_constant<int, 4>());
    }
    }
    update_t(M[1], std::integral_constant<int, 5>());
    update_y(5);
    asm volatile("s_waitcnt vmcnt(0) lgkmcnt(0)\n\ts_barrier" ::: "memory");

    if constexpr (INC == 3) {
        static_assert(WGM == 2 && WGN == 4 && NBUF == 3, "INC 3 is built for the 2 x 4 wave workgroup");
        constexpr int K2 = 128, ROWS2 = 128;
        constexpr int W2_FLOATS = ROWS2 * K2;
        constexpr int XB_FLOATS = NW * 512;
        constexpr int XPOS = MM_INC3_PAIR ? 2 : 1;
        static_assert((W2_FLOATS + 2 * XPOS * XB_FLOATS + 512) * 4 <= inc3_lds_bytes(NBUF * ROWS * KS * 4), "epilogue tenants fit");
        float* xb = lds + W2_FLOATS;
        float* b2s = xb + 2 * XPOS * XB_FLOATS;
        f32x4v b1[2];
#pragma unroll
        for (int cb = 0; cb < 2; ++cb) {
            const float4 t = p.bias ? *reinterpret_cast<const float4*>(p.bias + wn * 32 + cb * 16 + 4 * lg) : float4{0.f, 0.f, 0.f, 0.f};
            b1[cb] = f32x4v{t.x, t.y, t.z, t.w};
        }
        const int tpi = p.TH * p.TW;
        const int t = m_base + wm * 16 + l16;
        const bool tok = t < p.ntile;
        const int tt = tok ? t : 0;
        const int bimg = tt / tpi, rem = tt - bimg * tpi;
        const int ty = rem / p.TW, tx = rem - ty * p.TW;
        const int64_t pix0 = ((int64_t)bimg * p.H + 4 * ty) * p.W + 4 * tx;
        int wa[8], xr[3];
#pragma unroll
        for (int sidx = 0; sidx < 8; ++sidx) {
            const int src = sidx < 2 ? wn : (wn + 1 + (sidx - 2) / 2) & 3;
            const int qd = (src * 8 + (sidx & 1) * 4 + lg) ^ l16;
            wa[sidx] = (wn * 32 + l16) * K2 + (qd << 2);
        }
#pragma unroll
        for (int k = 0; k < 3; ++k) xr[k] = ((wm * 4 + ((wn + 1 + k) & 3)) * 8 + lg) * 64 + l16 * 4;
        const int x_own = (wave * 8 + lg) * 64 + l16 * 4;
        for (int i = tid; i < 512; i += NW * 64) b2s[i] = p.bias2[i];
#pragma unroll
        for (int pp = 0; pp < 4; ++pp)
#pragma unroll
            for (int qq = 0; qq < 4; ++qq)
#pragma unroll
                for (int cb = 0; cb < 2; ++cb)
#pragma unroll
                    for (int e = 0; e < 4; ++e) {
                        const float v = Y[pp][qq][cb][e] + b1[cb][e];
                        Y[pp][qq][cb][e] = p.relu ? fmaxf(v, 0.f) : v;
                    }
        for (int pass = 0; pass < 4; ++pass) {
            if (pass) asm volatile("s_waitcnt vmcnt(0) lgkmcnt(0)\n\ts_barrier" ::: "memory");
            {
                const __amdgpu_buffer_rsrc_t rw = __builtin_amdgcn_make_buffer_rsrc(const_cast<float*>(p.w2) + (int64_t)pass * W2_FLOATS, 0,
                                                                                    (unsigned)(W2_FLOATS * 4), 0x00020000);
#pragma unroll
                for (int it = 0; it < ROWS2 / (2 * NW); ++it) {
                    const int row = (it * NW + wave) * 2 + (lane >> 5);
                    const unsigned voff = (unsigned)(row * K2 + (((lane & 31) ^ (row & 15)) << 2)) * 4u;
                    dma1(rw, voff, lds0 + (unsigned)((it * NW + wave) * 1024));
                }
            }
            const int c0 = pass * 128 + wn * 32 + 4 * lg;
            const float* rbase = p.res + pix0 * p.C2 + c0;
            float* obase = p.out + pix0 * p.C2 + c0;
            auto res_rows = [&](f32x4v (&r)[2], int pos) {
                const int pp = pos >> 2, qq = pos & 3;
                const bool pok = tok && 4 * ty + pp < p.H && 4 * tx + qq < p.W;
                const float* rp = pok ? rbase + ((int64_t)pp * p.W + qq) * p.C2 : p.res + c0;
#pragma unroll
                for (int j = 0; j < 2; ++j) r[j] = *reinterpret_cast<const f32x4v*>(rp + j * 16);
            };
            f32x4v rs[2][2], Pr[3][2];
            res_rows(rs[0], 0);
            asm volatile("s_waitcnt vmcnt(0) lgkmcnt(0)\n\ts_barrier" ::: "memory");
#if MM_INC3_PAIR
#pragma unroll
            for (int pr = 0; pr < 8; ++pr) {
                float* xbuf = xb + (pr & 1) * 2 * XB_FLOATS;
#pragma unroll
                for (int h = 0; h < 2; ++h)
#pragma unroll
                    for (int cb = 0; cb < 2; ++cb)
                        *reinterpret_cast<f32x4v*>(xbuf + h * XB_FLOATS + x_own + cb * 256) = Y[(2 * pr + h) >> 2][(2 * pr + h) & 3][cb];
                asm volatile("s_waitcnt lgkmcnt(0)\n\ts_barrier" ::: "memory");
#pragma unroll
                for (int h = 0; h < 2; ++h) {
                    const int pos = 2 * pr + h, pp = pos >> 2, qq = pos & 3;
                    __builtin_amdgcn_sched_barrier(0);
#pragma unroll
                    for (int k = 0; k < 3; ++k)
#pragma unroll
                        for (int cb = 0; cb < 2; ++cb) Pr[k][cb] = *reinterpret_cast<const f32x4v*>(xbuf + h * XB_FLOATS + xr[k] + cb * 256);
                    if (pos + 1 < 16) res_rows(rs[(pos + 1) & 1], pos + 1);
                    f32x4v acc[2];
#pragma unroll
                    for (int j = 0; j < 2; ++j) acc[j] = *reinterpret_cast<const f32x4v*>(b2s + c0 + j * 16);
#pragma unroll
                    for (int sidx = 0; sidx < 8; ++sidx) {
                        const f32x4v Bv = sidx < 2 ? Y[pp][qq][sidx & 1] : Pr[(sidx - 2) >> 1][sidx & 1];
                        float4 w4[2];
#pragma unroll
                        for (int j = 0; j < 2; ++j) w4[j] = *reinterpret_cast<const float4*>(lds + wa[sidx] + (j * 16) * K2);
#pragma unroll
                        for (int j = 0; j < 2; ++j) acc[j] = __builtin_amdgcn_mfma_f32_16x16x4f32(w4[j].x, Bv[0], acc[j], 0, 0, 0);
#pragma unroll
                        for (int j = 0; j < 2; ++j) acc[j] = __builtin_amdgcn_mfma_f32_16x16x4f32(w4[j].y, Bv[1], acc[j], 0, 0, 0);
#pragma unroll
                        for (int j = 0; j < 2; ++j) acc[j] = __builtin_amdgcn_mfma_f32_16x16x4f32(w4[j].z, Bv[2], acc[j], 0, 0, 0);
#pragma unroll
                        for (int j = 0; j < 2; ++j) acc[j] = __builtin_amdgcn_mfma_f32_16x16x4f32(w4[j].w, Bv[3], acc[j], 0, 0, 0);
                    }
#pragma unroll
                    for (int j = 0; j < 2; ++j) {
                        acc[j] = acc[j] + rs[pos & 1][j];
#pragma unroll
                        for (int e = 0; e < 4; ++e) acc[j][e] = fmaxf(acc[j][e], 0.f);
                    }
                    if (tok && 4 * ty + pp < p.H && 4 * tx + qq < p.W) {
                        float* op = obase + ((int64_t)pp * p.W + qq) * p.C2;
#pragma unroll
                        for (int j = 0; j < 2; ++j) inc_store(acc[j], op + j * 16);
                    }
                }
            }
            continue;
#endif
#pragma unroll
            for (int pos = 0; pos < 16; ++pos) {
                const int pp = pos >> 2, qq = pos & 3;
                float* xbuf = xb + (pos & 1) * XB_FLOATS;
#pragma unroll
                for (int cb = 0; cb < 2; ++cb) *reinterpret_cast<f32x4v*>(xbuf + x_own + cb * 256) = Y[pp][qq][cb];
                asm volatile("s_waitcnt lgkmcnt(0)\n\ts_barrier" ::: "memory");
#pragma unroll
                for (int k = 0; k < 3; ++k)
#pragma unroll
                    for (int cb = 0; cb < 2; ++cb) Pr[k][cb] = *reinterpret_cast<const f32x4v*>(xbuf + xr[k] + cb * 256);
                if (pos + 1 < 16) res_rows(rs[(pos + 1) & 1], pos + 1);
                f32x4v acc[2];
#pragma unroll
                for (int j = 0; j < 2; ++j) acc[j] = *reinterpret_cast<const f32x4v*>(b2s + c0 + j * 16);
#pragma unroll
                for (int sidx = 0; sidx < 8; ++sidx) {
                    const f32x4v Bv = sidx < 2 ? Y[pp][qq][sidx & 1] : Pr[(sidx - 2) >> 1][sidx & 1];
                    float4 w4[2];
#pragma unroll
                    for (int j = 0; j < 2; ++j) w4[j] = *reinterpret_cast<const float4*>(lds + wa[sidx] + (j * 16) * K2);
#pragma unroll
                    for (int j = 0; j < 2; ++j) acc[j] = __builtin_amdgcn_mfma_f32_16x16x4f32(w4[j].x, Bv[0], acc[j], 0, 0, 0);
#pragma unroll
                    for (int j = 0; j < 2; ++j) acc[j] = __builtin_amdgcn_mfma_f32_16x16x4f32(w4[j].y, Bv[1], acc[j], 0, 0, 0);
#pragma unroll
                    for (int j = 0; j < 2; ++j) acc[j] = __builtin_amdgcn_mfma_f32_16x16x4f32(w4[j].z, Bv[2], acc[j], 0, 0, 0);
#pragma unroll
                    for (int j = 0; j < 2; ++j) acc[j] = __builtin_amdgcn_mfma_f32_16x16x4f32(w4[j].w, Bv[3], acc[j], 0, 0, 0);
                }
#pragma unroll
                for (int j = 0; j < 2; ++j) {
                    acc[j] = acc[j] + rs[pos & 1][j];
#pragma unroll
                    for (int e = 0; e < 4; ++e) acc[j][e] = fmaxf(acc[j][e], 0.f);
                }
                if (tok && 4 * ty + pp < p.H && 4 * tx + qq < p.W) {
                    float* op = obase + ((int64_t)pp * p.W + qq) * p.C2;
#pragma unroll
                    for (int j = 0; j < 2; ++j) inc_store(acc[j], op + j * 16);
                }
            }
        }
        return;
    }
    if constexpr (INC == 2) {
        static_assert(WGM == 2 && NBUF == 3, "INC is built for the four-wave workgroup");
        constexpr int K2 = 2 * KS;
        constexpr int W2_FLOATS = 128 * K2;
        float* xb = lds + W2_FLOATS;
        float* b2s = xb + 2048;
        const int x_own = (wave * 8 + lg) * 64 + l16 * 4, x_par = ((wave ^ 1) * 8 + lg) * 64 + l16 * 4;
        f32x4v b1[2];
#pragma unroll
        for (int cb = 0; cb < 2; ++cb) {
            const float4 t = p.bias ? *reinterpret_cast<const float4*>(p.bias + wn * 32 + cb * 16 + 4 * lg) : float4{0.f, 0.f, 0.f, 0.f};
            b1[cb] = f32x4v{t.x, t.y, t.z, t.w};
        }
        const int tpi = p.TH * p.TW;
        const int t = m_base + wm * 16 + l16;
        const bool tok = t < p.ntile;
        const int tt = tok ? t : 0;
        const int bimg = tt / tpi, rem = tt - bimg * tpi;
        const int ty = rem / p.TW, tx = rem - ty * p.TW;
        const int64_t pix0 = ((int64_t)bimg * p.H + 4 * ty) * p.W + 4 * tx;
        const float* xbase = p.res + pix0 * KS + 4 * lg;
        int wa[8];
#pragma unroll
        for (int sidx = 0; sidx < 8; ++sidx) {
            const int qd = sidx < 4 ? ((sidx < 2 ? wn : 1 - wn) * 8 + (sidx & 1) * 4 + lg) : 16 + (sidx - 4) * 4 + lg;
            wa[sidx] = (wn * 64 + l16) * K2 + ((qd ^ l16) << 2);
        }
        b2s[tid] = p.bias2[tid];
#pragma unroll
        for (int pp = 0; pp < 4; ++pp)
#pragma unroll
            for (int qq = 0; qq < 4; ++qq)
#pragma unroll
                for (int cb = 0; cb < 2; ++cb)
#pragma unroll
                    for (int e = 0; e < 4; ++e) {
                        const float v = Y[pp][qq][cb][e] + b1[cb][e];
                        Y[pp][qq][cb][e] = p.relu ? fmaxf(v, 0.f) : v;
                    }
        auto x_rows = [&](f32x4v (&r)[4], int pos) {
            const int pp = pos >> 2, qq = pos & 3;
            const bool pok = tok && 4 * ty + pp < p.H && 4 * tx + qq < p.W;
            const float* xp = pok ? xbase + ((int64_t)pp * p.W + qq) * KS : p.res + 4 * lg;
#pragma unroll
            for (int j = 0; j < 4; ++j) r[j] = *reinterpret_cast<const f32x4v*>(xp + j * 16);
        };
        for (int pass = 0; pass < 2; ++pass) {
            if (pass) asm volatile("s_waitcnt vmcnt(0) lgkmcnt(0)\n\ts_barrier" ::: "memory");
            {
                const __amdgpu_buffer_rsrc_t rw = __builtin_amdgcn_make_buffer_rsrc(const_cast<float*>(p.w2) + (int64_t)pass * W2_FLOATS, 0,
                                                                                    (unsigned)(W2_FLOATS * 4), 0x00020000);
#pragma unroll
                for (int it = 0; it < 128 / (2 * NW); ++it) {
                    const int row = (it * NW + wave) * 2 + (lane >> 5);
                    const unsigned voff = (unsigned)(row * K2 + (((lane & 31) ^ (row & 15)) << 2)) * 4u;
                    dma1(rw, voff, lds0 + (unsigned)((it * NW + wave) * 1024));
                }
            }
            const int c0 = pass * 128 + wn * 64 + 4 * lg;
            float* obase = p.out + pix0 * p.C2 + c0;
            f32x4v xs[2][4], Pr[2];
            x_rows(xs[0], 0);
            asm volatile("s_waitcnt vmcnt(0) lgkmcnt(0)\n\ts_barrier" ::: "memory");
#pragma unroll
            for (int pos = 0; pos < 16; ++pos) {
                const int pp = pos >> 2, qq = pos & 3;
                if (pos) asm volatile("s_waitcnt lgkmcnt(0)\n\ts_barrier" ::: "memory");
#pragma unroll
                for (int cb = 0; cb < 2; ++cb) *reinterpret_cast<f32x4v*>(xb + x_own + cb * 256) = Y[pp][qq][cb];
                asm volatile("s_waitcnt lgkmcnt(0)\n\ts_barrier" ::: "memory");
#pragma unroll
                for (int cb = 0; cb < 2; ++cb) Pr[cb] = *reinterpret_cast<const f32x4v*>(xb + x_par + cb * 256);
                if (pos + 1 < 16) x_rows(xs[(pos + 1) & 1], pos + 1);
                f32x4v acc[4];
#pragma unroll
                for (int j = 0; j < 4; ++j) acc[j] = *reinterpret_cast<const f32x4v*>(b2s + c0 + j * 16);
#pragma unroll
                for (int sidx = 0; sidx < 8; ++sidx) {
                    const f32x4v Bv = sidx < 2 ? Y[pp][qq][sidx & 1] : sidx < 4 ? Pr[sidx & 1] : xs[pos & 1][sidx - 4];
                    float4 w4[4];
#pragma unroll
                    for (int j = 0; j < 4; ++j) w4[j] = *reinterpret_cast<const float4*>(lds + wa[sidx] + (j * 16) * K2);
#pragma unroll
                    for (int j = 0; j < 4; ++j) acc[j] = __builtin_amdgcn_mfma_f32_16x16x4f32(w4[j].x, Bv[0], acc[j], 0, 0, 0);
#pragma unroll
                    for (int j = 0; j < 4; ++j) acc[j] = __builtin_amdgcn_mfma_f32_16x16x4f32(w4[j].y, Bv[1], acc[j], 0, 0, 0);
#pragma unroll
                    for (int j = 0; j < 4; ++j) acc[j] = __builtin_amdgcn_mfma_f32_16x16x4f32(w4[j].z, Bv[2], acc[j], 0, 0, 0);
#pragma unroll
                    for (int j = 0; j < 4; ++j) acc[j] = __builtin_amdgcn_mfma_f32_16x16x4f32(w4[j].w, Bv[3], acc[j], 0, 0, 0);
                }
#pragma unroll
                for (int j = 0; j < 4; ++j)
#pragma unroll
                    for (int e = 0; e < 4; ++e) acc[j][e] = fmaxf(acc[j][e], 0.f);
                if (tok && 4 * ty + pp < p.H && 4 * tx + qq < p.W) {
                    float* op = obase + ((int64_t)pp * p.W + qq) * p.C2;
#pragma unroll
                    for (int j = 0; j < 4; ++j) inc_store(acc[j], op + j * 16);
                }
            }
        }
        return;
    }
    if constexpr (INC == 1) {
        static_assert((WGM == 2 || WGM == 4) && WGN == 2 && NBUF == 3, "INC 1 is built for the four- and the eight-wave workgroup");
        constexpr int W2_FLOATS = 256 * KS;
        constexpr bool W3_REAL = NEXT && WGM == 4;
        {
            const __amdgpu_buffer_rsrc_t rw = __builtin_amdgcn_make_buffer_rsrc(const_cast<float*>(p.w2), 0, (unsigned)(W2_FLOATS * 4), 0x00020000);
#pragma unroll
            for (int it = 0; it < 256 / (4 * NW); ++it) {
                const int row = (it * NW + wave) * 4 + (lane >> 4);
                const unsigned voff = (unsigned)(row * KS + (((lane & 15) ^ (row & 15)) << 2)) * 4u;
                dma1(rw, voff, lds0 + (unsigned)((it * NW + wave) * 1024));
            }
        }
        float* xb = lds + W2_FLOATS;
        const int x_own = (wave * 8 + lg) * 64 + l16 * 4, x_par = ((wave ^ 1) * 8 + lg) * 64 + l16 * 4;
        float* b2s = xb + NW * 512;
        float* b3s = b2s + 256;
        float* w3s = b3s + 64;
        if constexpr (W3_REAL) {
            const __amdgpu_buffer_rsrc_t rw3 = __builtin_amdgcn_make_buffer_rsrc(const_cast<float*>(p.w3), 0, (unsigned)(64 * 256 * 4), 0x00020000);
            const unsigned w3b = lds0 + (unsigned)(W2_FLOATS + NW * 512 + 256 + 64) * 4u;
#pragma unroll
            for (int it = 0; it < 64 / NW; ++it) {
                const int row = it * NW + wave;
                const unsigned voff = (unsigned)(row * 256 + ((lane ^ (row & 15)) << 2)) * 4u;
                dma1(rw3, voff, w3b + (unsigned)(row * 1024));
            }
        }
        f32x4v b1[2];
#pragma unroll
        for (int cb = 0; cb < 2; ++cb) {
            const float4 t = p.bias ? *reinterpret_cast<const float4*>(p.bias + wn * 32 + cb * 16 + 4 * lg) : float4{0.f, 0.f, 0.f, 0.f};
            b1[cb] = f32x4v{t.x, t.y, t.z, t.w};
        }
        const int tpi = p.TH * p.TW;
        const int t = m_base + wm * 16 + l16;
        const bool tok = t < p.ntile;
        const int tt = tok ? t : 0;
        const int bimg = tt / tpi, rem = tt - bimg * tpi;
        const int ty = rem / p.TW, tx = rem - ty * p.TW;
        const int64_t pix0 = ((int64_t)bimg * p.H + 4 * ty) * p.W + 4 * tx;
        const int c0 = wn * 128 + 4 * lg;
        const float* rbase = p.res + pix0 * p.C2 + c0;
        float* obase = p.out + pix0 * p.C2 + c0;
        int wa[4];
#pragma unroll
        for (int sidx = 0; sidx < 4; ++sidx) {
            const int qd = ((sidx < 2 ? wn : 1 - wn) * 8 + (sidx & 1) * 4 + lg) ^ l16;
            wa[sidx] = (wn * 128 + l16) * KS + (qd << 2);
        }
        int w3a[4] = {0, 0, 0, 0};
        float* o3base = nullptr;
        if constexpr (NEXT) {
#pragma unroll
            for (int j = 0; j < 4; ++j) {
                if constexpr (W3_REAL) w3a[j] = l16 * 256 + (((32 * wn + 4 * j + lg) ^ l16) << 2);
                else w3a[j] = l16 * KS + (((4 * j + lg) ^ l16) << 2);
            }
            o3base = p.out3 + pix0 * 64 + 32 * wn + 4 * lg;
        }
        if (tid < 256) b2s[tid] = p.bias2[tid];
        if (NEXT && tid < 64) b3s[tid] = p.bias3[tid];
        asm volatile("s_waitcnt vmcnt(0) lgkmcnt(0)\n\ts_barrier" ::: "memory");
        auto res_rows = [&](f32x4v (&r)[4], int step) {
            const int pp = step >> 3, qq = (step >> 1) & 3, h = step & 1;
            const bool pok = tok && 4 * ty + pp < p.H && 4 * tx + qq < p.W;
#ifdef MM_MEASURE
            const float* rp = !pok ? p.res + c0
                              : (p.ablate & 2) ? p.res + ((pix0 + (int64_t)pp * p.W + qq) & 4095) * p.C2 + c0
                                               : rbase + ((int64_t)pp * p.W + qq) * p.C2;
#else
            const float* rp = pok ? rbase + ((int64_t)pp * p.W + qq) * p.C2 : p.res + c0;
#endif
#pragma unroll
            for (int j = 0; j < 4; ++j) r[j] = *reinterpret_cast<const f32x4v*>(rp + h * 64 + j * 16);
        };
#ifndef MM_INC1_RES_DEPTH
#define MM_INC1_RES_DEPTH 3
#endif
        auto res_ahead = [](int step) {
            if (step < 0) return 0;
            int d = 1 + ((NEXT ? (step < 4 ? 0 : step - 4) : step) >> 2);
            d = d > MM_INC1_RES_DEPTH ? MM_INC1_RES_DEPTH : d;
            const int t = step + d;
            return t > 31 ? 31 : t;
        };
        if constexpr (NEXT) {
#pragma unroll
            for (int pp = 0; pp < 4; ++pp)
#pragma unroll
                for (int qq = 0; qq < 4; ++qq)
#pragma unroll
                    for (int cb = 0; cb < 2; ++cb)
#pragma unroll
                        for (int e = 0; e < 4; ++e) {
                            const float v = Y[pp][qq][cb][e] + b1[cb][e];
                            Y[pp][qq][cb][e] = p.relu ? fmaxf(v, 0.f) : v;
                        }
        }
        f32x4v rs[4][4], Pr[2], D[4];
#ifdef MM_MEASURE
        const int abl = p.ablate;
#else
        constexpr int abl = 0;
#endif
        if (abl & 8) {
#pragma unroll
            for (int j = 0; j < 4; ++j) rs[0][j] = rs[1][j] = rs[2][j] = rs[3][j] = f32x4v{0.f, 0.f, 0.f, 0.f};
        } else
        res_rows(rs[0], 0);
#pragma unroll
        for (int step = 0; step < 32; ++step) {
            const int pp = step >> 3, qq = (step >> 1) & 3, h = step & 1;
            if (h == 0) {
                if constexpr (!NEXT) {
#pragma unroll
                for (int cb = 0; cb < 2; ++cb)
#pragma unroll
                    for (int e = 0; e < 4; ++e) {
                        const float v = Y[pp][qq][cb][e] + b1[cb][e];
                        Y[pp][qq][cb][e] = p.relu ? fmaxf(v, 0.f) : v;
                    }
                }
                if (!NEXT && step && !(abl & 32)) asm volatile("s_waitcnt lgkmcnt(0)\n\ts_barrier" ::: "memory");
#pragma unroll
                for (int cb = 0; cb < 2; ++cb) *reinterpret_cast<f32x4v*>(xb + x_own + cb * 256) = Y[pp][qq][cb];
                if (!(abl & 32)) asm volatile("s_waitcnt lgkmcnt(0)\n\ts_barrier" ::: "memory");
#pragma unroll
                for (int cb = 0; cb < 2; ++cb) Pr[cb] = *reinterpret_cast<const f32x4v*>(xb + x_par + cb * 256);
                if constexpr (NEXT) D[0] = D[1] = D[2] = D[3] = f32x4v{0.f, 0.f, 0.f, 0.f};
            }
            if (!(abl & 8)) {
#pragma unroll
                for (int t = res_ahead(step - 1) + 1; t <= res_ahead(step); ++t) res_rows(rs[t & 3], t);
            }
            f32x4v acc[4];
#pragma unroll
            for (int j = 0; j < 4; ++j) acc[j] = *reinterpret_cast<const f32x4v*>(b2s + c0 + h * 64 + j * 16);
            if (!(abl & 64))
#pragma unroll
            for (int sidx = 0; sidx < 4; ++sidx) {
                const f32x4v Bv = sidx < 2 ? Y[pp][qq][sidx & 1] : Pr[sidx & 1];
                float4 w4[4];
#pragma unroll
                for (int j = 0; j < 4; ++j) w4[j] = *reinterpret_cast<const float4*>(lds + wa[sidx] + (h * 64 + j * 16) * KS);
#pragma unroll
                for (int j = 0; j < 4; ++j) acc[j] = __builtin_amdgcn_mfma_f32_16x16x4f32(w4[j].x, Bv[0], acc[j], 0, 0, 0);
#pragma unroll
                for (int j = 0; j < 4; ++j) acc[j] = __builtin_amdgcn_mfma_f32_16x16x4f32(w4[j].y, Bv[1], acc[j], 0, 0, 0);
#pragma unroll
                for (int j = 0; j < 4; ++j) acc[j] = __builtin_amdgcn_mfma_f32_16x16x4f32(w4[j].z, Bv[2], acc[j], 0, 0, 0);
#pragma unroll
                for (int j = 0; j < 4; ++j) acc[j] = __builtin_amdgcn_mfma_f32_16x16x4f32(w4[j].w, Bv[3], acc[j], 0, 0, 0);
            }
#pragma unroll
            for (int j = 0; j < 4; ++j) {
                acc[j] = acc[j] + rs[step & 3][j];
#pragma unroll
                for (int e = 0; e < 4; ++e) acc[j][e] = fmaxf(acc[j][e], 0.f);
            }
            const bool pix_ok = tok && 4 * ty + pp < p.H && 4 * tx + qq < p.W;
            if (pix_ok && !(abl & 16)) {
                float* op = obase + ((int64_t)pp * p.W + qq) * p.C2 + h * 64;
#pragma unroll
                for (int j = 0; j < 4; ++j) inc_store(acc[j], op + j * 16);
            }
            if constexpr (NEXT) {
#pragma unroll
                for (int j = 0; j < 4; ++j) {
                    float4 w4[4];
#pragma unroll
                    for (int nb = 0; nb < 4; ++nb)
                        w4[nb] = *reinterpret_cast<const float4*>((W3_REAL ? w3s + nb * 16 * 256 + 16 * h * 4 : lds + (nb * 16 + h * 64) * KS) + w3a[j]);
#pragma unroll
                    for (int nb = 0; nb < 4; ++nb) D[nb] = __builtin_amdgcn_mfma_f32_16x16x4f32(w4[nb].x, acc[j][0], D[nb], 0, 0, 0);
#pragma unroll
                    for (int nb = 0; nb < 4; ++nb) D[nb] = __builtin_amdgcn_mfma_f32_16x16x4f32(w4[nb].y, acc[j][1], D[nb], 0, 0, 0);
#pragma unroll
                    for (int nb = 0; nb < 4; ++nb) D[nb] = __builtin_amdgcn_mfma_f32_16x16x4f32(w4[nb].z, acc[j][2], D[nb], 0, 0, 0);
#pragma unroll
                    for (int nb = 0; nb < 4; ++nb) D[nb] = __builtin_amdgcn_mfma_f32_16x16x4f32(w4[nb].w, acc[j][3], D[nb], 0, 0, 0);
                    __builtin_amdgcn_sched_barrier(0);
                }
                if (h == 1) {
                    f32x4v give[2], keep[2];
#pragma unroll
                    for (int i = 0; i < 2; ++i)
#pragma unroll
                        for (int e = 0; e < 4; ++e) {
                            const float lo = D[i][e], hi = D[2 + i][e];
                            give[i][e] = wn ? lo : hi;
                            keep[i][e] = wn ? hi : lo;
                        }
#pragma unroll
                    for (int i = 0; i < 2; ++i) *reinterpret_cast<f32x4v*>(xb + x_par + i * 256) = give[i];
                    asm volatile("s_waitcnt lgkmcnt(0)\n\ts_barrier" ::: "memory");
#pragma unroll
                    for (int i = 0; i < 2; ++i) {
                        const f32x4v got = *reinterpret_cast<const f32x4v*>(xb + x_own + i * 256);
                        f32x4v d = keep[i] + got + *reinterpret_cast<const f32x4v*>(b3s + 32 * wn + 16 * i + 4 * lg);
#pragma unroll
                        for (int e = 0; e < 4; ++e) d[e] = fmaxf(d[e], 0.f);
                        if (pix_ok && !(abl & 16)) __builtin_nontemporal_store(d, reinterpret_cast<f32x4v*>(o3base + ((int64_t)pp * p.W + qq) * 64 + i * 16));
                    }
                }
            }
        }
        return;
    }
    constexpr int SLD = 36;
    float* st = lds + wave * (16 * SLD);
    const int cq = lane & 7, tr = lane >> 3;
    const int n4 = n_base + wn * 32 + cq * 4;
    const bool nok = n4 < p.Cout;
    float4 bias4 = {0.f, 0.f, 0.f, 0.f};
    if (nok && p.bias) bias4 = *reinterpret_cast<const float4*>(p.bias + n4);
    const int tpi = p.TH * p.TW;
    int64_t obase[2];
    int ty4[2], tx4[2];
    bool tok[2];
#pragma unroll
    for (int g = 0; g < 2; ++g) {
        const int t = m_base + wm * 16 + g * 8 + tr;
        tok[g] = nok && t < p.ntile;
        const int tt = tok[g] ? t : 0;
        const int b = tt / tpi, rem = tt - b * tpi;
        const int ty = rem / p.TW, tx = rem - ty * p.TW;
        ty4[g] = 4 * ty;
        tx4[g] = 4 * tx;
        obase[g] = (((int64_t)b * p.H + 4 * ty) * p.W + 4 * tx) * p.Cout + n4;
    }
#pragma unroll
    for (int pp = 0; pp < 4; ++pp) {
#pragma unroll
        for (int qq = 0; qq < 4; ++qq) {
#pragma unroll
            for (int cb = 0; cb < 2; ++cb)
#pragma unroll
                for (int e = 0; e < 4; ++e) st[(4 * lg + e) * SLD + cb * 16 + l16] = Y[pp][qq][cb][e];
            __builtin_amdgcn_fence(__ATOMIC_RELEASE, "wavefront");
            float4 v[2];
#pragma unroll
            for (int g = 0; g < 2; ++g) v[g] = *reinterpret_cast<const float4*>(st + (g * 8 + tr) * SLD + cq * 4);
            __builtin_amdgcn_fence(__ATOMIC_ACQUIRE, "wavefront");
#pragma unroll
            for (int g = 0; g < 2; ++g) {
                if (!tok[g] || ty4[g] + pp >= p.H || tx4[g] + qq >= p.W) continue;
                float4 o = {v[g].x + bias4.x, v[g].y + bias4.y, v[g].z + bias4.z, v[g].w + bias4.w};
                if (p.relu) o = float4{fmaxf(o.x, 0.f), fmaxf(o.y, 0.f), fmaxf(o.z, 0.f), fmaxf(o.w, 0.f)};
                const f32x4v ov = {o.x, o.y, o.z, o.w};
                __builtin_nontemporal_store(ov, reinterpret_cast<f32x4v*>(p.out + obase[g] + ((int64_t)pp * p.W + qq) * p.Cout));
            }
        }
    }
}

template <int NBUF, int WGM, int INC = 0, int WGN = 2, int KSL = 0, int NEXT = 0>
static int launch_fused_k(WinoFusedParams p, hipStream_t s) {
    constexpr int BM = 16 * WGM, BN = 32 * WGN;
    constexpr int RING_BYTES = NBUF * (BM + BN) * 64 * 4;
    constexpr int EPI_BYTES = (INC == 1 || INC == 2) ? (256 * 64 + WGM * WGN * 512 + 256 + (NEXT ? 64 : 0) + (NEXT && WGM == 4 ? 64 * 256 : 0)) * 4 : 0;
    constexpr int LDS_BYTES = (INC == 1 || INC == 2) ? (EPI_BYTES > RING_BYTES ? EPI_BYTES : RING_BYTES)
                              : INC == 3 ? inc3_lds_bytes(RING_BYTES) : RING_BYTES;
    static_assert(LDS_BYTES >= RING_BYTES && LDS_BYTES <= 160 * 1024, "the ring must fit too");
    static bool attr_set[16] = {};
    int dev = 0;
    (void)hipGetDevice(&dev);
    if (dev >= 0 && dev < 16 && !attr_set[dev]) {
        MM_HIP(hipFuncSetAttribute(reinterpret_cast<const void*>(wino_fused_kernel<NBUF, WGM, INC, WGN, KSL, NEXT>), hipFuncAttributeMaxDynamicSharedMemorySize,
                                   LDS_BYTES));
        attr_set[dev] = true;
    }
#ifdef MM_MEASURE
    static const int lds_pad = getenv("MM_WF_LDS_PAD") ? atoi(getenv("MM_WF_LDS_PAD")) : 0;
    static const int ablate = getenv("MM_WF_ABLATE") ? atoi(getenv("MM_WF_ABLATE")) : 0;
    const int lds_bytes = LDS_BYTES + (INC ? lds_pad : 0);
    p.ablate = INC ? ablate : 0;
    if (INC && lds_pad)
        MM_HIP(hipFuncSetAttribute(reinterpret_cast<const void*>(wino_fused_kernel<NBUF, WGM, INC, WGN, KSL, NEXT>), hipFuncAttributeMaxDynamicSharedMemorySize,
                                   lds_bytes));
#else
    constexpr int lds_bytes = LDS_BYTES;
    p.ablate = 0;
#endif
    p.tiles_n = (p.Cout + BN - 1) / BN;
    for (int q = 0; q < 6; ++q)
        for (int qq = 0; qq < 4; ++qq) p.at_cols[q * 4 + qq] = kAtHost[qq][q];
    const int64_t blocks = (int64_t)((p.ntile + BM - 1) / BM) * p.tiles_n;
    if (blocks <= 0 || blocks > 0x7fffffff) return MM_ERR_INVALID_ARG;
    if (prof_enabled()) {
        char tag[64];
        snprintf(tag, sizeof(tag), "wino-fused%s%s M=%d K=%d N=%d t%dx%d b36", INC == 3 ? "+inc512" : INC == 2 ? "+incproj256" : INC ? "+inc256" : "",
                 NEXT ? "+red64" : "", p.ntile, p.K, p.Cout, BM, BN);
        double fl = 2.0 * 36.0 * (double)p.ntile * (double)p.K * (double)p.Cout;
        if (INC) fl += 2.0 * (double)p.B * p.H * p.W * (double)(INC == 2 ? 2 * p.Cout : p.Cout) * (double)p.C2;
        if (NEXT) fl += 2.0 * (double)p.B * p.H * p.W * (double)p.C2 * 64.0;
        prof_before(0, fl, s, tag);
    }
    hipLaunchKernelGGL((wino_fused_kernel<NBUF, WGM, INC, WGN, KSL, NEXT>), dim3((unsigned)blocks), dim3(WGM * WGN * 64), lds_bytes, s, p);
    prof_after(0, s);
    MM_LAUNCH_CHECK();
    return MM_OK;
}

template <int NBUF, int WGM, int INC = 0, int WGN = 2, int NEXT = 0>
static int launch_fused(const WinoFusedParams& p, hipStream_t s) {
    if constexpr (INC == 1 && (NEXT || WGM == 4)) {
        if (p.K != 64) return MM_ERR_UNSUPPORTED;
        return p.generic_loop ? launch_fused_k<NBUF, WGM, INC, WGN, 0, NEXT>(p, s) : launch_fused_k<NBUF, WGM, INC, WGN, 1, NEXT>(p, s);
    } else {
    if constexpr (NBUF == 3 && WGM == 2 && WGN == 4 && INC == 3) {
        if (!p.generic_loop && p.K == 128) return launch_fused_k<NBUF, WGM, INC, WGN, 2>(p, s);
    }
    if constexpr (NBUF == 3 && WGM * WGN == 4) {
        if (!p.generic_loop && p.K == 64) return launch_fused_k<NBUF, WGM, INC, WGN, 1>(p, s);
        if constexpr (INC == 0) {
            if (!p.generic_loop && p.K == 128) return launch_fused_k<NBUF, WGM, INC, WGN, 2>(p, s);
            if (!p.generic_loop && p.K == 256) return launch_fused_k<NBUF, WGM, INC, WGN, 4>(p, s);
        }
    }
    return launch_fused_k<NBUF, WGM, INC, WGN, 0>(p, s);
    }
}

bool wino_fused_supported(int64_t ntile, int Cin, int Cout) {
    if (Cin <= 0 || Cout <= 0 || Cin % 64 || Cout % 32) return false;
    return (ntile + 64) * Cin * 4 < 0xFFFFF000ll && ((int64_t)Cout + 64) * Cin * 4 < 0xFFFFF000ll;
}

bool wino_fused_inc_supported(int64_t ntile, int Cin, int Cout, int C2) {
    return ((Cout == 64 && C2 == 256) || (Cout == 128 && C2 == 512)) && wino_fused_supported(ntile, Cin, Cout);
}

int wino_gemm_output_fused(const float* V, const float* U, const float* bias, float* y, int B, int H, int W, int Cin, int Cout,
                            int relu, int shape, hipStream_t s, int generic_loop) {
    WinoFusedParams p;
    p.generic_loop = generic_loop;
    p.V = V; p.U = U; p.bias = bias; p.out = y;
    p.w2 = nullptr; p.bias2 = nullptr; p.res = nullptr; p.C2 = 0;
    p.w3 = nullptr; p.bias3 = nullptr; p.out3 = nullptr;
    p.TH = (H + 3) / 4; p.TW = (W + 3) / 4;
    const int64_t ntile = (int64_t)B * p.TH * p.TW;
    if (!wino_fused_supported(ntile, Cin, Cout)) return MM_ERR_UNSUPPORTED;
    if (ntile <= 0) return MM_OK;
    p.ntile = (int)ntile; p.K = Cin; p.Cout = Cout; p.B = B; p.H = H; p.W = W; p.relu = relu; p.tiles_n = 0;
    return shape == 4 ? launch_fused<4, 4>(p, s) : shape == 8 ? launch_fused<3, 4>(p, s) : launch_fused<3, 2>(p, s);
}

int wino_gemm_output_fused_inc(const float* V, const float* U, const float* bias, const float* W2, const float* bias2, const float* res,
                               float* out, int B, int H, int W, int Cin, int Cout, int C2, int relu, hipStream_t s, int generic_loop,
                               const float* next_w, const float* next_bias, float* next_out, int shape) {
    if (!V || !U || !W2 || !bias2 || !res || !out) return MM_ERR_INVALID_ARG;
    WinoFusedParams p;
    p.generic_loop = generic_loop;
    p.V = V; p.U = U; p.bias = bias; p.out = out;
    p.w2 = W2; p.bias2 = bias2; p.res = res; p.C2 = C2;
    p.w3 = nullptr; p.bias3 = nullptr; p.out3 = nullptr;
    p.TH = (H + 3) / 4; p.TW = (W + 3) / 4;
    const int64_t ntile = (int64_t)B * p.TH * p.TW;
    if (!wino_fused_inc_supported(ntile, Cin, Cout, C2)) return MM_ERR_UNSUPPORTED;
    if (ntile <= 0) return MM_OK;
    p.ntile = (int)ntile; p.K = Cin; p.Cout = Cout; p.B = B; p.H = H; p.W = W; p.relu = relu; p.tiles_n = 0;
    if (Cout == 128) return next_w ? MM_ERR_UNSUPPORTED : launch_fused<3, 2, 3, 4>(p, s);
    if (next_w) {
        if (!next_bias || !next_out || C2 != 256) return MM_ERR_INVALID_ARG;
        p.w3 = next_w; p.bias3 = next_bias; p.out3 = next_out;
#ifdef MM_MEASURE
        if (shape == 2) return launch_fused<3, 2, 1, 2, 1>(p, s);
#endif
        return launch_fused<3, 4, 1, 2, 1>(p, s);
    }
    if (shape == 8) return launch_fused<3, 4, 1>(p, s);
    return launch_fused<3, 2, 1>(p, s);
}

int wino_gemm_output_fused_incproj(const float* V, const float* U, const float* bias, const float* W2, const float* bias2, const float* x,
                                   float* out, int B, int H, int W, int Cin, int Cout, int C2, int relu, hipStream_t s, int generic_loop) {
    if (!V || !U || !W2 || !bias2 || !x || !out) return MM_ERR_INVALID_ARG;
    WinoFusedParams p;
    p.generic_loop = generic_loop;
    p.V = V; p.U = U; p.bias = bias; p.out = out;
    p.w2 = W2; p.bias2 = bias2; p.res = x; p.C2 = C2;
    p.w3 = nullptr; p.bias3 = nullptr; p.out3 = nullptr;
    p.TH = (H + 3) / 4; p.TW = (W + 3) / 4;
    const int64_t ntile = (int64_t)B * p.TH * p.TW;
    if (Cout != 64 || !wino_fused_inc_supported(ntile, Cin, Cout, C2)) return MM_ERR_UNSUPPORTED;
    if (ntile <= 0) return MM_OK;
    p.ntile = (int)ntile; p.K = Cin; p.Cout = Cout; p.B = B; p.H = H; p.W = W; p.relu = relu; p.tiles_n = 0;
    return launch_fused<3, 2, 2>(p, s);
}

}
```

Baseline: 21000.

## Compute only stride-2 output pixels in fused Winograd+increase kernel before downsample

Adds a SUB2 variant of the fused Winograd 3x3 + 1x1 increase kernel. When the following block downsamples by stride 2, it builds only the even output positions of each 4x4 tile (2x2 per tile), needing 5 of the 6 transform rows/cols. It writes a half-resolution output directly, skipping output-transform, increase-GEMM and residual work plus stores for pixels the next stride-2 layer would drop. It is enabled by default through fuse_inc=4. Separately, the Python package now sets GPU_MAX_HW_QUEUES to at least 8 at import time.

After: 21890, median of 6. 1.04x the previous value.

```diff
diff --git a/mimamo-net_amd/__init__.py b/mimamo-net_amd/__init__.py
--- a/mimamo-net_amd/__init__.py
+++ b/mimamo-net_amd/__init__.py
@@ -1,4 +1,25 @@
+import os
+
 __version__ = "0.1.0"
+
+_HW_QUEUES = 8
+
+
+def _ensure_hw_queues(environ=os.environ):
+    knob = environ.get("MM_HW_QUEUES")
+    try:
+        if knob is not None:
+            n = int(knob)
+            if n > 0:
+                environ["GPU_MAX_HW_QUEUES"] = str(min(n, 32))
+        elif int(environ.get("GPU_MAX_HW_QUEUES", "0")) < _HW_QUEUES:
+            environ["GPU_MAX_HW_QUEUES"] = str(_HW_QUEUES)
+    except ValueError:
+        pass
+    return environ.get("GPU_MAX_HW_QUEUES")
+
+
+_ensure_hw_queues()
 
 _LAZY = {
     "Phase_Difference_Extractor": ".phase_difference_extractor",
diff --git a/mimamo-net_amd/csrc/conv.h b/mimamo-net_amd/csrc/conv.h
--- a/mimamo-net_amd/csrc/conv.h
+++ b/mimamo-net_amd/csrc/conv.h
@@ -59,7 +59,8 @@
                            int relu, int shape, hipStream_t s, int generic_loop = 0);
 int wino_gemm_output_fused_inc(const float* V, const float* U, const float* bias, const float* W2, const float* bias2, const float* res,
                                float* out, int B, int H, int W, int Cin, int Cout, int C2, int relu, hipStream_t s, int generic_loop = 0,
-                               const float* next_w = nullptr, const float* next_bias = nullptr, float* next_out = nullptr, int shape = 0);
+                               const float* next_w = nullptr, const float* next_bias = nullptr, float* next_out = nullptr, int shape = 0,
+                               int sub2 = 0);
 bool wino_fused_inc_supported(int64_t ntile, int Cin, int Cout, int C2);
 int wino_gemm_output_fused_incproj(const float* V, const float* U, const float* bias, const float* W2, const float* bias2, const float* x,
                                    float* out, int B, int H, int W, int Cin, int Cout, int C2, int relu, hipStream_t s, int generic_loop = 0);
diff --git a/mimamo-net_amd/csrc/nets.hip b/mimamo-net_amd/csrc/nets.hip
--- a/mimamo-net_amd/csrc/nets.hip
+++ b/mimamo-net_amd/csrc/nets.hip
@@ -209,7 +209,8 @@
 static int run_layer_wino(const Layer& L, const float* in, int B, int H, int W, float* out, float* V, float* M, int m, hipStream_t s,
                           const Layer* inc = nullptr, const float* inc_res = nullptr, float* inc_out = nullptr, bool inc_two_src = false,
                           int x3 = 0, int generic_loop = 0, int no_sched = 0, const Layer* next = nullptr, float* next_out = nullptr,
-                          int inc_shape = 0) {
+                          int inc_shape = 0, bool* sub2_done = nullptr) {
+    if (sub2_done) *sub2_done = false;
     const int mt = m == 5 ? 4 : m;
     const int TH = (H + mt - 1) / mt, TW = (W + mt - 1) / mt, npos = (mt + 2) * (mt + 2);
     const int64_t ntile = (int64_t)B * TH * TW;
@@ -230,6 +231,12 @@
     if (inc && inc_two_src)
         return wino_gemm_output_fused_incproj(V, L.wino_u4, L.bias, inc->w, inc->bias, inc_res, inc_out, B, H, W, wc, L.cout, inc->cout,
                                               L.relu, s, generic_loop);
+    if (inc && sub2_done) {
+        rc = wino_gemm_output_fused_inc(V, L.wino_u4, L.bias, inc->w, inc->bias, inc_res, inc_out, B, H, W, wc, L.cout, inc->cout, L.relu, s,
+                                        generic_loop, next ? next->w : nullptr, next ? next->bias : nullptr, next_out, inc_shape, 1);
+        *sub2_done = rc == MM_OK;
+        if (rc != MM_ERR_UNSUPPORTED) return rc;
+    }
     if (inc)
         return wino_gemm_output_fused_inc(V, L.wino_u4, L.bias, inc->w, inc->bias, inc_res, inc_out, B, H, W, wc, L.cout, inc->cout,
                                           L.relu, s, generic_loop, next ? next->w : nullptr, next ? next->bias : nullptr, next_out, inc_shape);
@@ -421,7 +428,7 @@
         const char* fpl = getenv("MM_FUSE_POOL");
         h->fuse_pool = fpl ? atoi(fpl) : 2;
         const char* fi = getenv("MM_FUSE_INC");
-        h->fuse_inc = fi ? atoi(fi) : 3;
+        h->fuse_inc = fi ? atoi(fi) : 4;
         const char* fn = getenv("MM_FUSE_NEXT");
         h->fuse_next = fn ? atoi(fn) : 0;
         const char* is = getenv("MM_INC1_SHAPE");
@@ -635,12 +642,13 @@
         }
         const int wm_ = h->winograd == 1 ? (Bk.conv3.cin <= g_wino_fused_max_cin ? 5 : 4) : h->winograd;
         const int wt_ = wm_ == 5 ? 4 : wm_;
-        bool inc_done = false;
+        bool inc_done = false, inc_sub2 = false;
         if (wm_ && Bk.conv3.wino_u &&
             (int64_t)(wt_ + 2) * (wt_ + 2) * ((H1 + wt_ - 1) / wt_) * ((W1 + wt_ - 1) / wt_) * Bk.conv3.cin <= kRsWino) {
             rc = MM_ERR_UNSUPPORTED;
             if (wm_ == 5 && h->fuse_inc && !Bk.has_proj && !tail_unfuse && (Bk.conv3.cout == 64 || h->fuse_inc >= 3)) {
                 const bool nx = h->fuse_next && Bk.conv3.cout == 64 && Nx && !Nx->has_proj && Nx->reduce.stride == 1;
+                bool* const s2 = tail && h->fuse_inc >= 4 ? &inc_sub2 : nullptr;
                 if (nx) {
                     rc = run_layer_wino(Bk.conv3, y1, B, H1, W1, nullptr, wv, nullptr, 5, s, &Bk.increase, x, o, false, 0, h->wf_generic, 0, &Nx->reduce, y1,
                                         h->inc_shape);
@@ -648,7 +656,7 @@
                 }
                 if (!nx || rc == MM_ERR_UNSUPPORTED)
                     rc = run_layer_wino(Bk.conv3, y1, B, H1, W1, nullptr, wv, nullptr, 5, s, &Bk.increase, x, o, false, 0, h->wf_generic, 0, nullptr, nullptr,
-                                        h->inc_shape);
+                                        h->inc_shape, s2);
                 inc_done = rc == MM_OK;
             } else if (wm_ == 5 && h->fuse_inc >= 2 && dual && Bk.proj_stride == 1 && C == Bk.conv3.cout && H1 == H && W1 == W) {
                 rc = run_layer_wino(Bk.conv3, y1, B, H1, W1, nullptr, wv, nullptr, 5, s, &Bk.inc_proj, x, o, true, 0, h->wf_generic);
@@ -660,7 +668,9 @@
             rc = run_layer(Bk.conv3, y1, B, H1, W1, Bk.reduce.cout, 0, y2, Bk.conv3.cout, 0, nullptr, 0, s, &H2, &W2, 0, ns);
         }
         if (rc != MM_OK) return rc;
-        if (inc_done) {
+        if (inc_done && inc_sub2) {
+            H3 = (H2 + 1) / 2; W3 = (W2 + 1) / 2;
+        } else if (inc_done) {
             H3 = H2; W3 = W2;
             tail = false;
         } else if (dual) {
diff --git a/mimamo-net_amd/csrc/wino_fused.hip b/mimamo-net_amd/csrc/wino_fused.hip
--- a/mimamo-net_amd/csrc/wino_fused.hip
+++ b/mimamo-net_amd/csrc/wino_fused.hip
@@ -1,6 +1,7 @@
 #include <cstdio>
 #include <cstdlib>
 #include <type_traits>
+#include <utility>
 #include "conv.h"
 
 namespace mm {
@@ -39,12 +40,22 @@
     return MM_INC3_PAIR && ring_bytes < (128 * 128 + 4 * 8 * 512 + 512) * 4 ? (128 * 128 + 4 * 8 * 512 + 512) * 4 : ring_bytes;
 }
 
+template <class F, int... I>
+__device__ __forceinline__ void for_ints(F&& f, std::integer_sequence<int, I...>) {
+    (f(std::integral_constant<int, I>()), ...);
+}
+
 __device__ constexpr float kAt[4][6] = {{1, 1, 1, 1, 1, 0}, {0, 1, -1, 2, -2, 0}, {0, 1, 1, 4, 4, 0}, {0, 1, -1, 8, -8, 1}};
 static constexpr float kAtHost[4][6] = {{1, 1, 1, 1, 1, 0}, {0, 1, -1, 2, -2, 0}, {0, 1, 1, 4, 4, 0}, {0, 1, -1, 8, -8, 1}};
 
-template <int NBUF, int WGM, int INC = 0, int WGN = 2, int KSL = 0, int NEXT = 0>
+template <int NBUF, int WGM, int INC = 0, int WGN = 2, int KSL = 0, int NEXT = 0, int SUB2 = 0>
 __global__ void __launch_bounds__(WGM * WGN * 64) __attribute__((amdgpu_waves_per_eu(2, 2)))
 wino_fused_kernel(const WinoFusedParams p) {
+    static_assert(!SUB2 || ((INC == 1 || INC == 3) && !NEXT && WGM == 2), "SUB2 exists for the four-wave INC 1 and the INC 3 shape");
+    constexpr int NP = SUB2 ? 2 : 4;
+    constexpr int PS = SUB2 ? 2 : 1;
+    constexpr int NQ = SUB2 ? 5 : 6;
+    constexpr int NR = SUB2 ? 5 : 6;
     constexpr int NW = WGN * WGM, BM = 16 * WGM, BN = 32 * WGN, KS = 64;
     constexpr int ROWS = BM + BN;
     constexpr int NIA = BM / (4 * NW), NIB = BN / (4 * NW);
@@ -89,7 +100,7 @@
     const char* pv = reinterpret_cast<const char*>(p.V);
     const char* pu = reinterpret_cast<const char*>(p.U);
     const int64_t step_a = 6 * (int64_t)plane_a, step_b = 6 * (int64_t)plane_b;
-    const int64_t back_a = 35 * (int64_t)plane_a, back_b = 35 * (int64_t)plane_b;
+    const int64_t back_a = (6 * NR - 1) * (int64_t)plane_a, back_b = (6 * NR - 1) * (int64_t)plane_b;
     unsigned rec_a = plane_a, rec_b = plane_b;
     unsigned koff = 0;
     int d_q = 0, d_r = 0, d_ks = 0, d_buf = 0;
@@ -144,11 +155,11 @@
             koff = 0;
             pv += step_a;
             pu += step_b;
-            if (++d_r == 6) {
+            if (++d_r == NR) {
                 d_r = 0;
                 pv -= back_a;
                 pu -= back_b;
-                if (++d_q == 6) rec_a = rec_b = 0;
+                if (++d_q == NQ) rec_a = rec_b = 0;
             }
         }
         d_buf = d_buf == NBUF - 1 ? 0 : d_buf + 1;
@@ -163,22 +174,22 @@
         fb1[j] = (BM + wn * 32 + 16 + l16) * KS + sw;
     }
 
-    f32x4v Y[4][4][2], T[4][2], M[2][2];
-#pragma unroll
-    for (int a = 0; a < 4; ++a)
+    f32x4v Y[NP][NP][2], T[NP][2], M[2][2];
+#pragma unroll
+    for (int a = 0; a < NP; ++a)
 #pragma unroll
         for (int c = 0; c < 2; ++c) {
             T[a][c] = f32x4v{0.f, 0.f, 0.f, 0.f};
 #pragma unroll
-            for (int b = 0; b < 4; ++b) Y[a][b][c] = f32x4v{0.f, 0.f, 0.f, 0.f};
+            for (int b = 0; b < NP; ++b) Y[a][b][c] = f32x4v{0.f, 0.f, 0.f, 0.f};
         }
     M[0][0] = M[0][1] = M[1][0] = M[1][1] = f32x4v{0.f, 0.f, 0.f, 0.f};
 
     auto update_t = [&](const f32x4v (&Mx)[2], auto rtag) {
         constexpr int r = decltype(rtag)::value;
 #pragma unroll
-        for (int pp = 0; pp < 4; ++pp) {
-            const float c = kAt[pp][r];
+        for (int pp = 0; pp < NP; ++pp) {
+            const float c = kAt[PS * pp][r];
             if (c == 0.f) continue;
 #pragma unroll
             for (int cb = 0; cb < 2; ++cb)
@@ -188,17 +199,17 @@
     };
     auto update_y = [&](int qc) {
 #pragma unroll
-        for (int qq = 0; qq < 4; ++qq) {
-            const float c = p.at_cols[qc * 4 + qq];
-#pragma unroll
-            for (int pp = 0; pp < 4; ++pp)
+        for (int qq = 0; qq < NP; ++qq) {
+            const float c = p.at_cols[qc * 4 + PS * qq];
+#pragma unroll
+            for (int pp = 0; pp < NP; ++pp)
 #pragma unroll
                 for (int cb = 0; cb < 2; ++cb)
 #pragma unroll
                     for (int e = 0; e < 4; ++e) Y[pp][qq][cb][e] = fmaf(c, T[pp][cb][e], Y[pp][qq][cb][e]);
         }
 #pragma unroll
-        for (int pp = 0; pp < 4; ++pp)
+        for (int pp = 0; pp < NP; ++pp)
 #pragma unroll
             for (int cb = 0; cb < 2; ++cb) T[pp][cb] = f32x4v{0.f, 0.f, 0.f, 0.f};
     };
@@ -271,8 +282,8 @@
         const unsigned dbase = __builtin_amdgcn_readfirstlane(lds0 + (unsigned)wave * 1024u);
         int dq = 0;
         auto dma_c = [&](auto d_tag) {
-            constexpr int D = decltype(d_tag)::value % NSL;
-            constexpr int DBUF = D % NBUF, DKS = D % KSL, DR = D / KSL;
+            constexpr int D = SUB2 ? decltype(d_tag)::value : decltype(d_tag)::value % NSL;
+            constexpr int DBUF = D % NBUF, DKS = D % KSL, DR = (D / KSL) % NR;
             constexpr unsigned SB = DBUF * SLAB_BYTES;
             const __amdgpu_buffer_rsrc_t ra = __builtin_amdgcn_make_buffer_rsrc(const_cast<char*>(pv), 0, rec_a, 0x00020000);
             const __amdgpu_buffer_rsrc_t rb = __builtin_amdgcn_make_buffer_rsrc(const_cast<char*>(pu), 0, rec_b, 0x00020000);
@@ -326,10 +337,10 @@
             if constexpr (DKS == KSL - 1) {
                 pv += step_a;
                 pu += step_b;
-                if constexpr (DR == 5) {
+                if constexpr (DR == NR - 1) {
                     pv -= back_a;
                     pu -= back_b;
-                    if (++dq == 6) rec_a = rec_b = 0;
+                    if (++dq == NQ) rec_a = rec_b = 0;
                 }
             }
         };
@@ -420,7 +431,31 @@
         };
         dma_c(std::integral_constant<int, 0>());
         dma_c(std::integral_constant<int, 1>());
-        for (int q = 0; q < 6; ++q) {
+        if constexpr (SUB2) {
+            auto anchor_t = [&]() {
+#pragma unroll
+                for (int pp = 0; pp < NP; ++pp) asm volatile("" : "+v"(T[pp][0]), "+v"(T[pp][1]));
+            };
+            auto anchor_y = [&]() {
+#pragma unroll
+                for (int pp = 0; pp < NP; ++pp)
+#pragma unroll
+                    for (int qq = 0; qq < NP; ++qq) asm volatile("" : "+v"(Y[pp][qq][0]), "+v"(Y[pp][qq][1]));
+            };
+            for_ints([&](auto p_tag) {
+                constexpr int P = decltype(p_tag)::value;
+                slab_c(std::integral_constant<int, P * KSL>(), nothing);
+                if constexpr (KSL > 1) slab_c(std::integral_constant<int, P * KSL + 1>(), nothing);
+                static_assert(KSL <= 2, "SUB2 runs at K = 64 and K = 128");
+                if constexpr (P > 0) {
+                    update_t(M[(P - 1) & 1], std::integral_constant<int, (P - 1) % 5>());
+                    if constexpr ((P - 1) % 5 == 4) update_y((P - 1) / 5);
+                    anchor_t();
+                    if constexpr ((P - 1) % 5 == 4) anchor_y();
+                }
+            }, std::make_integer_sequence<int, 25>());
+        } else
+        for (int q = 0; q < NQ; ++q) {
             if constexpr (MM_WF_HOOK && INC == 0) {
             position(std::integral_constant<int, 0>(), [&]() { update_t(M[1], std::integral_constant<int, 5>()); update_y(q == 0 ? 0 : q - 1); });
             position(std::integral_constant<int, 1>(), [&]() { update_t(M[0], std::integral_constant<int, 0>()); });
@@ -459,6 +494,26 @@
     } else {
 #pragma unroll
     for (int i = 0; i < NBUF - 1; ++i) dma_next();
+    if constexpr (SUB2) {
+        for (int q = 0; q < NQ; ++q) {
+            slab(M[0], std::true_type());
+            for (int ks = 1; ks < kslabs; ++ks) slab(M[0], std::false_type());
+            update_t(M[0], std::integral_constant<int, 0>());
+            slab(M[1], std::true_type());
+            for (int ks = 1; ks < kslabs; ++ks) slab(M[1], std::false_type());
+            update_t(M[1], std::integral_constant<int, 1>());
+            slab(M[0], std::true_type());
+            for (int ks = 1; ks < kslabs; ++ks) slab(M[0], std::false_type());
+            update_t(M[0], std::integral_constant<int, 2>());
+            slab(M[1], std::true_type());
+            for (int ks = 1; ks < kslabs; ++ks) slab(M[1], std::false_type());
+            update_t(M[1], std::integral_constant<int, 3>());
+            slab(M[0], std::true_type());
+            for (int ks = 1; ks < kslabs; ++ks) slab(M[0], std::false_type());
+            update_t(M[0], std::integral_constant<int, 4>());
+            update_y(q);
+        }
+    } else
     for (int q = 0; q < 6; ++q) {
         slab(M[0], std::true_type());
         for (int ks = 1; ks < kslabs; ++ks) slab(M[0], std::false_type());
@@ -481,8 +536,15 @@
         update_t(M[0], std::integral_constant<int, 4>());
     }
     }
-    update_t(M[1], std::integral_constant<int, 5>());
-    update_y(5);
+    if constexpr (SUB2) {
+        if constexpr (KSL > 0) {
+            update_t(M[0], std::integral_constant<int, 4>());
+            update_y(NQ - 1);
+        }
+    } else {
+        update_t(M[1], std::integral_constant<int, 5>());
+        update_y(5);
+    }
     asm volatile("s_waitcnt vmcnt(0) lgkmcnt(0)\n\ts_barrier" ::: "memory");
 
     if constexpr (INC == 3) {
@@ -507,6 +569,9 @@
         const int bimg = tt / tpi, rem = tt - bimg * tpi;
         const int ty = rem / p.TW, tx = rem - ty * p.TW;
         const int64_t pix0 = ((int64_t)bimg * p.H + 4 * ty) * p.W + 4 * tx;
+        constexpr int NPOS = NP * NP;
+        const int OW = SUB2 ? (p.W + 1) / 2 : p.W;
+        const int64_t opix0 = SUB2 ? ((int64_t)bimg * ((p.H + 1) / 2) + 2 * ty) * OW + 2 * tx : pix0;
         int wa[8], xr[3];
 #pragma unroll
         for (int sidx = 0; sidx < 8; ++sidx) {
@@ -519,9 +584,9 @@
         const int x_own = (wave * 8 + lg) * 64 + l16 * 4;
         for (int i = tid; i < 512; i += NW * 64) b2s[i] = p.bias2[i];
 #pragma unroll
-        for (int pp = 0; pp < 4; ++pp)
-#pragma unroll
-            for (int qq = 0; qq < 4; ++qq)
+        for (int pp = 0; pp < NP; ++pp)
+#pragma unroll
+            for (int qq = 0; qq < NP; ++qq)
 #pragma unroll
                 for (int cb = 0; cb < 2; ++cb)
 #pragma unroll
@@ -543,11 +608,11 @@
             }
             const int c0 = pass * 128 + wn * 32 + 4 * lg;
             const float* rbase = p.res + pix0 * p.C2 + c0;
-            float* obase = p.out + pix0 * p.C2 + c0;
+            float* obase = p.out + opix0 * p.C2 + c0;
             auto res_rows = [&](f32x4v (&r)[2], int pos) {
-                const int pp = pos >> 2, qq = pos & 3;
-                const bool pok = tok && 4 * ty + pp < p.H && 4 * tx + qq < p.W;
-                const float* rp = pok ? rbase + ((int64_t)pp * p.W + qq) * p.C2 : p.res + c0;
+                const int pp = pos / NP, qq = pos % NP;
+                const bool pok = tok && 4 * ty + PS * pp < p.H && 4 * tx + PS * qq < p.W;
+                const float* rp = pok ? rbase + ((int64_t)(PS * pp) * p.W + PS * qq) * p.C2 : p.res + c0;
 #pragma unroll
                 for (int j = 0; j < 2; ++j) r[j] = *reinterpret_cast<const f32x4v*>(rp + j * 16);
             };
@@ -556,23 +621,23 @@
             asm volatile("s_waitcnt vmcnt(0) lgkmcnt(0)\n\ts_barrier" ::: "memory");
 #if MM_INC3_PAIR
 #pragma unroll
-            for (int pr = 0; pr < 8; ++pr) {
+            for (int pr = 0; pr < NPOS / 2; ++pr) {
                 float* xbuf = xb + (pr & 1) * 2 * XB_FLOATS;
 #pragma unroll
                 for (int h = 0; h < 2; ++h)
 #pragma unroll
                     for (int cb = 0; cb < 2; ++cb)
-                        *reinterpret_cast<f32x4v*>(xbuf + h * XB_FLOATS + x_own + cb * 256) = Y[(2 * pr + h) >> 2][(2 * pr + h) & 3][cb];
+                        *reinterpret_cast<f32x4v*>(xbuf + h * XB_FLOATS + x_own + cb * 256) = Y[(2 * pr + h) / NP][(2 * pr + h) % NP][cb];
                 asm volatile("s_waitcnt lgkmcnt(0)\n\ts_barrier" ::: "memory");
 #pragma unroll
                 for (int h = 0; h < 2; ++h) {
-                    const int pos = 2 * pr + h, pp = pos >> 2, qq = pos & 3;
+                    const int pos = 2 * pr + h, pp = pos / NP, qq = pos % NP;
                     __builtin_amdgcn_sched_barrier(0);
 #pragma unroll
                     for (int k = 0; k < 3; ++k)
 #pragma unroll
                         for (int cb = 0; cb < 2; ++cb) Pr[k][cb] = *reinterpret_cast<const f32x4v*>(xbuf + h * XB_FLOATS + xr[k] + cb * 256);
-                    if (pos + 1 < 16) res_rows(rs[(pos + 1) & 1], pos + 1);
+                    if (pos + 1 < NPOS) res_rows(rs[(pos + 1) & 1], pos + 1);
                     f32x4v acc[2];
 #pragma unroll
                     for (int j = 0; j < 2; ++j) acc[j] = *reinterpret_cast<const f32x4v*>(b2s + c0 + j * 16);
@@ -597,8 +662,8 @@
 #pragma unroll
                         for (int e = 0; e < 4; ++e) acc[j][e] = fmaxf(acc[j][e], 0.f);
                     }
-                    if (tok && 4 * ty + pp < p.H && 4 * tx + qq < p.W) {
-                        float* op = obase + ((int64_t)pp * p.W + qq) * p.C2;
+                    if (tok && 4 * ty + PS * pp < p.H && 4 * tx + PS * qq < p.W) {
+                        float* op = obase + ((int64_t)pp * OW + qq) * p.C2;
 #pragma unroll
                         for (int j = 0; j < 2; ++j) inc_store(acc[j], op + j * 16);
                     }
@@ -607,8 +672,8 @@
             continue;
 #endif
 #pragma unroll
-            for (int pos = 0; pos < 16; ++pos) {
-                const int pp = pos >> 2, qq = pos & 3;
+            for (int pos = 0; pos < NPOS; ++pos) {
+                const int pp = pos / NP, qq = pos % NP;
                 float* xbuf = xb + (pos & 1) * XB_FLOATS;
 #pragma unroll
                 for (int cb = 0; cb < 2; ++cb) *reinterpret_cast<f32x4v*>(xbuf + x_own + cb * 256) = Y[pp][qq][cb];
@@ -617,7 +682,7 @@
                 for (int k = 0; k < 3; ++k)
 #pragma unroll
                     for (int cb = 0; cb < 2; ++cb) Pr[k][cb] = *reinterpret_cast<const f32x4v*>(xbuf + xr[k] + cb * 256);
-                if (pos + 1 < 16) res_rows(rs[(pos + 1) & 1], pos + 1);
+                if (pos + 1 < NPOS) res_rows(rs[(pos + 1) & 1], pos + 1);
                 f32x4v acc[2];
 #pragma unroll
                 for (int j = 0; j < 2; ++j) acc[j] = *reinterpret_cast<const f32x4v*>(b2s + c0 + j * 16);
@@ -642,8 +707,8 @@
 #pragma unroll
                     for (int e = 0; e < 4; ++e) acc[j][e] = fmaxf(acc[j][e], 0.f);
                 }
-                if (tok && 4 * ty + pp < p.H && 4 * tx + qq < p.W) {
-                    float* op = obase + ((int64_t)pp * p.W + qq) * p.C2;
+                if (tok && 4 * ty + PS * pp < p.H && 4 * tx + PS * qq < p.W) {
+                    float* op = obase + ((int64_t)pp * OW + qq) * p.C2;
 #pragma unroll
                     for (int j = 0; j < 2; ++j) inc_store(acc[j], op + j * 16);
                 }
@@ -796,9 +861,12 @@
         const int bimg = tt / tpi, rem = tt - bimg * tpi;
         const int ty = rem / p.TW, tx = rem - ty * p.TW;
         const int64_t pix0 = ((int64_t)bimg * p.H + 4 * ty) * p.W + 4 * tx;
+        constexpr int NSTEP = 2 * NP * NP;
+        const int OW = (p.W + 1) / 2;
         const int c0 = wn * 128 + 4 * lg;
         const float* rbase = p.res + pix0 * p.C2 + c0;
         float* obase = p.out + pix0 * p.C2 + c0;
+        if constexpr (SUB2) obase = p.out + (((int64_t)bimg * ((p.H + 1) / 2) + 2 * ty) * OW + 2 * tx) * p.C2 + c0;
         int wa[4];
 #pragma unroll
         for (int sidx = 0; sidx < 4; ++sidx) {
@@ -819,7 +887,7 @@
         if (NEXT && tid < 64) b3s[tid] = p.bias3[tid];
         asm volatile("s_waitcnt vmcnt(0) lgkmcnt(0)\n\ts_barrier" ::: "memory");
         auto res_rows = [&](f32x4v (&r)[4], int step) {
-            const int pp = step >> 3, qq = (step >> 1) & 3, h = step & 1;
+            const int pp = SUB2 ? 2 * (step >> 2) : step >> 3, qq = SUB2 ? 2 * ((step >> 1) & 1) : (step >> 1) & 3, h = step & 1;
             const bool pok = tok && 4 * ty + pp < p.H && 4 * tx + qq < p.W;
 #ifdef MM_MEASURE
             const float* rp = !pok ? p.res + c0
@@ -835,6 +903,7 @@
 #define MM_INC1_RES_DEPTH 3
 #endif
         auto res_ahead = [](int step) {
+            if constexpr (SUB2) return step + 3 > NSTEP - 1 ? NSTEP - 1 : step + 3;
             if (step < 0) return 0;
             int d = 1 + ((NEXT ? (step < 4 ? 0 : step - 4) : step) >> 2);
             d = d > MM_INC1_RES_DEPTH ? MM_INC1_RES_DEPTH : d;
@@ -843,9 +912,9 @@
         };
         if constexpr (NEXT) {
 #pragma unroll
-            for (int pp = 0; pp < 4; ++pp)
-#pragma unroll
-                for (int qq = 0; qq < 4; ++qq)
+            for (int pp = 0; pp < NP; ++pp)
+#pragma unroll
+                for (int qq = 0; qq < NP; ++qq)
 #pragma unroll
                     for (int cb = 0; cb < 2; ++cb)
 #pragma unroll
@@ -863,11 +932,14 @@
         if (abl & 8) {
 #pragma unroll
             for (int j = 0; j < 4; ++j) rs[0][j] = rs[1][j] = rs[2][j] = rs[3][j] = f32x4v{0.f, 0.f, 0.f, 0.f};
+        } else if constexpr (SUB2) {
+#pragma unroll
+            for (int t = 0; t <= res_ahead(-1); ++t) res_rows(rs[t & 3], t);
         } else
         res_rows(rs[0], 0);
 #pragma unroll
-        for (int step = 0; step < 32; ++step) {
-            const int pp = step >> 3, qq = (step >> 1) & 3, h = step & 1;
+        for (int step = 0; step < NSTEP; ++step) {
+            const int pp = SUB2 ? step >> 2 : step >> 3, qq = SUB2 ? (step >> 1) & 1 : (step >> 1) & 3, h = step & 1;
             if (h == 0) {
                 if constexpr (!NEXT) {
 #pragma unroll
@@ -915,9 +987,9 @@
 #pragma unroll
                 for (int e = 0; e < 4; ++e) acc[j][e] = fmaxf(acc[j][e], 0.f);
             }
-            const bool pix_ok = tok && 4 * ty + pp < p.H && 4 * tx + qq < p.W;
+            const bool pix_ok = tok && 4 * ty + PS * pp < p.H && 4 * tx + PS * qq < p.W;
             if (pix_ok && !(abl & 16)) {
-                float* op = obase + ((int64_t)pp * p.W + qq) * p.C2 + h * 64;
+                float* op = obase + ((int64_t)pp * (SUB2 ? OW : p.W) + qq) * p.C2 + h * 64;
 #pragma unroll
                 for (int j = 0; j < 4; ++j) inc_store(acc[j], op + j * 16);
             }
@@ -1011,7 +1083,7 @@
     }
 }
 
-template <int NBUF, int WGM, int INC = 0, int WGN = 2, int KSL = 0, int NEXT = 0>
+template <int NBUF, int WGM, int INC = 0, int WGN = 2, int KSL = 0, int NEXT = 0, int SUB2 = 0>
 static int launch_fused_k(WinoFusedParams p, hipStream_t s) {
     constexpr int BM = 16 * WGM, BN = 32 * WGN;
     constexpr int RING_BYTES = NBUF * (BM + BN) * 64 * 4;
@@ -1023,7 +1095,7 @@
     int dev = 0;
     (void)hipGetDevice(&dev);
     if (dev >= 0 && dev < 16 && !attr_set[dev]) {
-        MM_HIP(hipFuncSetAttribute(reinterpret_cast<const void*>(wino_fused_kernel<NBUF, WGM, INC, WGN, KSL, NEXT>), hipFuncAttributeMaxDynamicSharedMemorySize,
+        MM_HIP(hipFuncSetAttribute(reinterpret_cast<const void*>(wino_fused_kernel<NBUF, WGM, INC, WGN, KSL, NEXT, SUB2>), hipFuncAttributeMaxDynamicSharedMemorySize,
                                    LDS_BYTES));
         attr_set[dev] = true;
     }
@@ -1033,7 +1105,7 @@
     const int lds_bytes = LDS_BYTES + (INC ? lds_pad : 0);
     p.ablate = INC ? ablate : 0;
     if (INC && lds_pad)
-        MM_HIP(hipFuncSetAttribute(reinterpret_cast<const void*>(wino_fused_kernel<NBUF, WGM, INC, WGN, KSL, NEXT>), hipFuncAttributeMaxDynamicSharedMemorySize,
+        MM_HIP(hipFuncSetAttribute(reinterpret_cast<const void*>(wino_fused_kernel<NBUF, WGM, INC, WGN, KSL, NEXT, SUB2>), hipFuncAttributeMaxDynamicSharedMemorySize,
                                    lds_bytes));
 #else
     constexpr int lds_bytes = LDS_BYTES;
@@ -1046,21 +1118,34 @@
     if (blocks <= 0 || blocks > 0x7fffffff) return MM_ERR_INVALID_ARG;
     if (prof_enabled()) {
         char tag[64];
-        snprintf(tag, sizeof(tag), "wino-fused%s%s M=%d K=%d N=%d t%dx%d b36", INC == 3 ? "+inc512" : INC == 2 ? "+incproj256" : INC ? "+inc256" : "",
-                 NEXT ? "+red64" : "", p.ntile, p.K, p.Cout, BM, BN);
-        double fl = 2.0 * 36.0 * (double)p.ntile * (double)p.K * (double)p.Cout;
-        if (INC) fl += 2.0 * (double)p.B * p.H * p.W * (double)(INC == 2 ? 2 * p.Cout : p.Cout) * (double)p.C2;
+        constexpr int NPOS = SUB2 ? 25 : 36;
+        const double npix = SUB2 ? (double)p.B * ((p.H + 1) / 2) * ((p.W + 1) / 2) : (double)p.B * p.H * p.W;
+        snprintf(tag, sizeof(tag), "wino-fused%s%s%s M=%d K=%d N=%d t%dx%d b%d", INC == 3 ? "+inc512" : INC == 2 ? "+incproj256" : INC ? "+inc256" : "",
+                 NEXT ? "+red64" : "", SUB2 ? " sub2" : "", p.ntile, p.K, p.Cout, BM, BN, NPOS);
+        double fl = 2.0 * NPOS * (double)p.ntile * (double)p.K * (double)p.Cout;
+        if (INC) fl += 2.0 * npix * (double)(INC == 2 ? 2 * p.Cout : p.Cout) * (double)p.C2;
         if (NEXT) fl += 2.0 * (double)p.B * p.H * p.W * (double)p.C2 * 64.0;
         prof_before(0, fl, s, tag);
     }
-    hipLaunchKernelGGL((wino_fused_kernel<NBUF, WGM, INC, WGN, KSL, NEXT>), dim3((unsigned)blocks), dim3(WGM * WGN * 64), lds_bytes, s, p);
+    hipLaunchKernelGGL((wino_fused_kernel<NBUF, WGM, INC, WGN, KSL, NEXT, SUB2>), dim3((unsigned)blocks), dim3(WGM * WGN * 64), lds_bytes, s, p);
     prof_after(0, s);
     MM_LAUNCH_CHECK();
     return MM_OK;
 }
 
 template <int NBUF, int WGM, int INC = 0, int WGN = 2, int NEXT = 0>
-static int launch_fused(const WinoFusedParams& p, hipStream_t s) {
+static int launch_fused(const WinoFusedParams& p, hipStream_t s, int sub2 = 0) {
+    if (sub2) {
+        if constexpr (NBUF == 3 && WGM == 2 && WGN == 2 && INC == 1 && !NEXT) {
+            if (p.K != 64) return MM_ERR_UNSUPPORTED;
+            return p.generic_loop ? launch_fused_k<NBUF, WGM, INC, WGN, 0, 0, 1>(p, s) : launch_fused_k<NBUF, WGM, INC, WGN, 1, 0, 1>(p, s);
+        } else if constexpr (NBUF == 3 && WGM == 2 && WGN == 4 && INC == 3 && !NEXT) {
+            if (p.K != 128) return MM_ERR_UNSUPPORTED;
+            return p.generic_loop ? launch_fused_k<NBUF, WGM, INC, WGN, 0, 0, 1>(p, s) : launch_fused_k<NBUF, WGM, INC, WGN, 2, 0, 1>(p, s);
+        } else {
+            return MM_ERR_UNSUPPORTED;
+        }
+    }
     if constexpr (INC == 1 && (NEXT || WGM == 4)) {
         if (p.K != 64) return MM_ERR_UNSUPPORTED;
         return p.generic_loop ? launch_fused_k<NBUF, WGM, INC, WGN, 0, NEXT>(p, s) : launch_fused_k<NBUF, WGM, INC, WGN, 1, NEXT>(p, s);
@@ -1105,7 +1190,7 @@
 
 int wino_gemm_output_fused_inc(const float* V, const float* U, const float* bias, const float* W2, const float* bias2, const float* res,
                                float* out, int B, int H, int W, int Cin, int Cout, int C2, int relu, hipStream_t s, int generic_loop,
-                               const float* next_w, const float* next_bias, float* next_out, int shape) {
+                               const float* next_w, const float* next_bias, float* next_out, int shape, int sub2) {
     if (!V || !U || !W2 || !bias2 || !res || !out) return MM_ERR_INVALID_ARG;
     WinoFusedParams p;
     p.generic_loop = generic_loop;
@@ -1117,7 +1202,8 @@
     if (!wino_fused_inc_supported(ntile, Cin, Cout, C2)) return MM_ERR_UNSUPPORTED;
     if (ntile <= 0) return MM_OK;
     p.ntile = (int)ntile; p.K = Cin; p.Cout = Cout; p.B = B; p.H = H; p.W = W; p.relu = relu; p.tiles_n = 0;
-    if (Cout == 128) return next_w ? MM_ERR_UNSUPPORTED : launch_fused<3, 2, 3, 4>(p, s);
+    if (sub2 && (next_w || shape == 8)) return MM_ERR_UNSUPPORTED;
+    if (Cout == 128) return next_w ? MM_ERR_UNSUPPORTED : launch_fused<3, 2, 3, 4>(p, s, sub2);
     if (next_w) {
         if (!next_bias || !next_out || C2 != 256) return MM_ERR_INVALID_ARG;
         p.w3 = next_w; p.bias3 = next_bias; p.out3 = next_out;
@@ -1127,7 +1213,7 @@
         return launch_fused<3, 4, 1, 2, 1>(p, s);
     }
     if (shape == 8) return launch_fused<3, 4, 1>(p, s);
-    return launch_fused<3, 2, 1>(p, s);
+    return launch_fused<3, 2, 1>(p, s, sub2);
 }
 
 int wino_gemm_output_fused_incproj(const float* V, const float* U, const float* bias, const float* W2, const float* bias2, const float* x,
```
